# cxjyxxme/deep-online-video-stabilization

Measured on AMD Instinct MI355X. Metric: stabilized frames/sec (720p, before_ch=31), higher is better.
Workload: dtype f32 (bf16x3 split MFMA, f32 accumulate); 1 GPU; BASELINE.json configs[1]: v2_93 net, 1280x720, 1 stream(s)/GPU, batch=1 per stream, 13-ch stack from a 32-deep ring (lags 1,2,4,8,16,32; --before-ch 31 ignored as in the reference), ResNet-v2-50 regressor + 4x4 multi-grid warp + feedback; one independent stream set per GPU (replicas only); height=720, width=1280, streams_per_gpu=1, refine=1, operand_mode=4, launches_per_frame=64, hip_graph=True

## Files before the change

### deep-online-video-stabilization_amd/csrc/conv.hip

```cpp
#include "conv.h"
#include "prof.h"
#include <climits>
#include <cstdlib>
#include <algorithm>
#include <vector>

#include "conv_kernel.h"
#include "conv_ring_kernel.h"
#include "conv_b2b_kernel.h"

template <int PAIR>
__device__ __forceinline__ void conv_splitk_reduce_body(const ConvArgs& p, const ConvPair& pr) {
    const size_t q = (size_t)blockIdx.x * 256 + threadIdx.x;
    const int c4n = p.Cout / 4;
    if (q >= (size_t)p.M * c4n) return;
    const int m = (int)(q / c4n);
    const int n = (int)(q - (size_t)m * c4n) * 4;
    const bool t1 = PAIR && m >= pr.m_tower;
    const size_t slab = (size_t)p.M * p.Cout;
    const float* src = p.partial + (size_t)m * p.Cout + n;
    float4 s = *reinterpret_cast<const float4*>(src);
    for (int z = 1; z < p.splitk; ++z) {
        const float4 t = *reinterpret_cast<const float4*>(src + z * slab);
        s.x += t.x; s.y += t.y; s.z += t.z; s.w += t.w;
    }
    if (p.bias != nullptr) {
        const float4 b = *reinterpret_cast<const float4*>(p.bias + n);
        s.x += b.x; s.y += b.y; s.z += b.z; s.w += b.w;
    }
    if (p.residual != nullptr) {
        size_t ri;
        if (p.res_stride == 1 && p.res_H == p.Ho && p.res_W == p.Wo) {
            ri = (size_t)m * p.res_ld + n;
        } else {
            const int img = sn_fastdiv(m, p.div_hw_mul, p.div_hw_shift);
            const int rr = m - img * (p.Ho * p.Wo);
            const int oy = sn_fastdiv(rr, p.div_w_mul, p.div_w_shift), ox = rr - oy * p.Wo;
            ri = (((size_t)img * p.res_H + oy * p.res_stride) * p.res_W + ox * p.res_stride) * p.res_ld + n;
        }
        const float4 t = *reinterpret_cast<const float4*>(p.residual + (t1 ? pr.dres : 0) + ri);
        s.x += t.x; s.y += t.y; s.z += t.z; s.w += t.w;
    }
    if (p.out_scale != nullptr) {
        const float4 a = *reinterpret_cast<const float4*>(p.out_scale + n), b = *reinterpret_cast<const float4*>(p.out_shift + n);
        s.x = __builtin_fmaf(s.x, a.x, b.x); s.y = __builtin_fmaf(s.y, a.y, b.y);
        s.z = __builtin_fmaf(s.z, a.z, b.z); s.w = __builtin_fmaf(s.w, a.w, b.w);
    }
    if (p.out_scale != nullptr && p.out_floor != nullptr) {
        const float4 f = *reinterpret_cast<const float4*>(p.out_floor + n);
        s.x = fmaxf(s.x, f.x); s.y = fmaxf(s.y, f.y); s.z = fmaxf(s.z, f.z); s.w = fmaxf(s.w, f.w);
    } else if (p.relu_out) {
        s.x = fmaxf(s.x, 0.f); s.y = fmaxf(s.y, 0.f); s.z = fmaxf(s.z, 0.f); s.w = fmaxf(s.w, 0.f);
    }
    *reinterpret_cast<float4*>(p.y + (t1 ? pr.dy : 0) + (size_t)m * p.Cout + n) = s;
}
__global__ __launch_bounds__(256) void conv_splitk_reduce_kernel(const ConvArgs p) {
    conv_splitk_reduce_body<0>(p, ConvPair{});
}
__global__ __launch_bounds__(256) void conv_splitk_reduce_pair_kernel(const ConvArgs p, const ConvPair pr) {
    conv_splitk_reduce_body<1>(p, pr);
}

enum TileId { T128x128 = 0, T128x64 = 1, T64x64 = 2 };

static void tile_dims(int t, int& bm, int& bn) {
    bm = (t == T64x64) ? 64 : 128;
    bn = (t == T128x128) ? 128 : 64;
}

static int env_int(const char* name, int dflt) {
    const char* v = getenv(name);
    return v ? atoi(v) : dflt;
}

static int g_force_tile = -2, g_force_split = -1, g_force_bk16 = 0;

static int conv_bk(const ConvArgs& a) { return (a.rowrun || (a.Cin % 32 == 0 && !g_force_bk16)) ? 32 : 16; }
static int conv_total_steps(const ConvArgs& a) {
    if (a.rowrun) return a.KH * cdiv(a.KW * a.Cin, 32);
    return a.KH * a.KW * (a.Cin / conv_bk(a));
}

struct TuneEntry { int M, Cout, K, KH, ring, splitk; };
#include "conv_tuning_table.h"
#include "conv_tuning_table_packed.h"
static int g_tuning_profile = 0;
static std::vector<TuneEntry> g_tuning_runtime;
static int g_tuning_use_builtin = -1;

static int tuning_lookup(int M, int Cout, int K, int KH, int ring) {
    for (const TuneEntry& e : g_tuning_runtime)
        if (e.M == M && e.Cout == Cout && e.K == K && e.KH == KH && e.ring == ring) return e.splitk;
    if (g_tuning_use_builtin < 0) g_tuning_use_builtin = env_int("STABNET_CONV_TUNING_TABLE", 1);
    if (g_tuning_use_builtin && g_tuning_profile == 1)
        for (const TuneEntry& e : g_tuning_packed)
            if (e.M == M && e.Cout == Cout && e.K == K && e.KH == KH && e.ring == ring) return e.splitk;
    if (g_tuning_use_builtin)
        for (const TuneEntry& e : g_tuning_builtin)
            if (e.M == M && e.Cout == Cout && e.K == K && e.KH == KH && e.ring == ring) return e.splitk;
    return 0;
}

static int pick_tile(const ConvArgs& a, int& splitk) {
    if (g_force_tile == -2) {
        g_force_tile = env_int("STABNET_CONV_TILE", -1);
        g_force_split = env_int("STABNET_CONV_SPLITK", -1);
        g_force_bk16 = env_int("STABNET_CONV_BK16", 0);
    }
    const int force_tile = g_force_tile, force_split = g_force_split;
    if (force_tile >= 0) {
        const int steps0 = conv_total_steps(a);
        splitk = force_split > 0 ? std::min(force_split, steps0) : 1;
        return force_tile;
    }
    const int total_steps = conv_total_steps(a);
    const long blocks = (long)cdiv(a.M, 64) * cdiv(a.Cout, 64);
    const bool ring_path = a.rowrun || (a.in_scale_expected == 0 && a.up == 1 && a.Cin % 32 == 0);
    int s = tuning_lookup(a.M, a.Cout, a.K, a.KH, ring_path ? 1 : 0);
    static const int thr = env_int("STABNET_CONV_SPLIT_BELOW", 400), target = env_int("STABNET_CONV_SPLIT_TARGET", 448);
    if (s > 0) {
        s = std::min(s, std::max(1, total_steps / 2));
    } else if (blocks < thr && a.Cout % 4 == 0) {
        s = (int)((target + blocks / 2) / blocks);
        s = std::min(s, std::max(1, total_steps / 8));
        s = std::min(s, 32);
    } else {
        s = 1;
    }
    splitk = std::max(1, s);
    return T64x64;
}

size_t conv_plan(ConvArgs& a) {
    static const int swz = env_int("STABNET_CONV_XCD", 1);
    a.xcd_swizzle = swz;
    a.M = a.N * a.Ho * a.Wo;
    a.K = a.rowrun ? a.KH * 32 * cdiv(a.KW * a.Cin, 32) : a.KH * a.KW * a.Cin;
    if (a.x_ld == 0) a.x_ld = a.Cin;
    if (a.res_ld == 0) a.res_ld = a.Cout;
    sn_fastdiv_make((unsigned)(a.Ho * a.Wo), a.div_hw_mul, a.div_hw_shift);
    sn_fastdiv_make((unsigned)a.Wo, a.div_w_mul, a.div_w_shift);
    int splitk = 1;
    (void)pick_tile(a, splitk);
    const int total_steps = conv_total_steps(a);
    a.steps_per_split = cdiv(total_steps, splitk);
    a.splitk = cdiv(total_steps, a.steps_per_split);
    return a.splitk > 1 ? (size_t)a.splitk * a.M * a.Cout * sizeof(float) : 0;
}

template <int BM, int BN, int BK, int WM, int WN, int MODE, int NBUF, int BF16 = 0>
static int launch_one_nb(const ConvArgs& a, hipStream_t st) {
    constexpr size_t lds_op = NBUF * (size_t)(BM + BN) * (BK + 4) * sizeof(float);
    constexpr size_t lds_epi = 4 * (size_t)SN_EPI_WAVE_BYTES;
    constexpr size_t lds = lds_op > lds_epi ? lds_op : lds_epi;
    static bool configured = false;
    auto kern = conv_igemm_f32_kernel<BM, BN, BK, WM, WN, MODE, NBUF, BF16>;
    if (!configured) {
        if (lds > 64 * 1024) {
            hipError_t e = hipFuncSetAttribute(reinterpret_cast<const void*>(kern),
                                               hipFuncAttributeMaxDynamicSharedMemorySize, (int)lds);
            if (e != hipSuccess) {
                stabnet_set_error("conv: hipFuncSetAttribute(%zu B LDS) failed: %s", lds, hipGetErrorString(e));
                return STABNET_ERR_LAUNCH;
            }
        }
        configured = true;
    }
    dim3 grid(cdiv(a.M, BM), cdiv(a.Cout, BN), a.splitk);
    kern<<<grid, 256, lds, st>>>(a);
    SN_LAUNCH_CHECK("conv_igemm_f32_kernel");
    return STABNET_OK;
}

static thread_local int g_bf16_operands = 0;

static void igemm_variant(const ConvArgs& a, int bm, int bn, int bk, int mode, int& nbuf_out, int& bf16_out) {
    static const int nbuf = env_int("STABNET_CONV_NBUF", 0);
    bf16_out = (g_bf16_operands && bm == 64 && bn == 64 && bk == 32) ? g_bf16_operands : 0;
    const bool one_stage = nbuf == 1 || (nbuf == 0 && mode == 0 && bm == 64 && bn == 64 && a.M >= 32768);
    nbuf_out = (bf16_out != 1 && one_stage) ? 1 : 2;
}

template <int BM, int BN, int BK, int WM, int WN, int MODE>
static int launch_one_t(const ConvArgs& a, hipStream_t st) {
    int nbuf, bf16;
    igemm_variant(a, BM, BN, BK, MODE, nbuf, bf16);
    if constexpr (BM == 64 && BN == 64 && BK == 32) {
        if (bf16 == 1) return launch_one_nb<BM, BN, BK, WM, WN, MODE, 2, 1>(a, st);
        else if (bf16 == 2) return nbuf == 1 ? launch_one_nb<BM, BN, BK, WM, WN, MODE, 1, 2>(a, st) : launch_one_nb<BM, BN, BK, WM, WN, MODE, 2, 2>(a, st);
        else if (bf16 == 3) return nbuf == 1 ? launch_one_nb<BM, BN, BK, WM, WN, MODE, 1, 3>(a, st) : launch_one_nb<BM, BN, BK, WM, WN, MODE, 2, 3>(a, st);
    }
    return nbuf == 1 ? launch_one_nb<BM, BN, BK, WM, WN, MODE, 1>(a, st) : launch_one_nb<BM, BN, BK, WM, WN, MODE, 2>(a, st);
}

template <int BM, int BN, int BK, int WM, int WN>
static int launch_one(const ConvArgs& a, hipStream_t st) {
    if (a.up > 1) return launch_one_t<BM, BN, BK, WM, WN, 2>(a, st);
    if (a.pad == 0) return launch_one_t<BM, BN, BK, WM, WN, 0>(a, st);
    return launch_one_t<BM, BN, BK, WM, WN, 1>(a, st);
}

static int g_ring = -1;

static bool ring_eligible(const ConvArgs& a, int tile, bool has_prologue) {
    if (g_ring < 0) {
        g_ring = env_int("STABNET_CONV_RING", 1);
    }
    if (a.rowrun) return true;
    static const int lowk = env_int("STABNET_CONV_LOWK_IGEMM", 1);
    if (lowk && a.KH == 1 && a.KW == 1 && a.Cin == 64 && a.x_ld == a.Cin && a.out_floor == nullptr) return false;
    return g_ring && tile == T64x64 && !has_prologue && a.up == 1 && a.Cin % 32 == 0 && !g_force_bk16;
}
static bool ring_eligible(const ConvArgs& a, int tile) { return ring_eligible(a, tile, a.in_scale != nullptr); }

static int g_ring_wgs = 0;
static int g_ring_cus = 0;
static int g_reserved_cus = 0;
static int usable_cus(int cus) { return std::max(cus / 8, cus - std::max(0, g_reserved_cus)); }
static int ring_grid_cap() { return g_ring_cus > 0 ? g_ring_wgs / g_ring_cus * usable_cus(g_ring_cus) : g_ring_wgs; }

template <int MODE>
static int launch_ring_mode(const ConvArgs& a, hipStream_t st) {
    if (g_ring_wgs == 0) {
        int dev = 0, cus = 0;
        if (hipGetDevice(&dev) != hipSuccess || hipDeviceGetAttribute(&cus, hipDeviceAttributeMultiprocessorCount, dev) != hipSuccess ||
            cus <= 0) {
            stabnet_set_error("conv: cannot read the CU count");
            return STABNET_ERR_LAUNCH;
        }
        g_ring_wgs = env_int("STABNET_CONV_RING_WGS_PER_CU", 3) * cus;
        g_ring_cus = cus;
    }
    const long ntiles = (long)cdiv(a.M, 64) * cdiv(a.Cout, 64) * a.splitk;
    const int grid = (int)std::min<long>(ntiles, ring_grid_cap());
    if (g_bf16_operands == 1) conv_ring_f32_kernel<MODE, 1><<<grid, 256, 0, st>>>(a);
    else if (g_bf16_operands == 2) conv_ring_f32_kernel<MODE, 2><<<grid, 256, 0, st>>>(a);
    else if (g_bf16_operands == 3) conv_ring_f32_kernel<MODE, 3><<<grid, 256, 0, st>>>(a);
    else conv_ring_f32_kernel<MODE, 0><<<grid, 256, 0, st>>>(a);
    SN_LAUNCH_CHECK("conv_ring_f32_kernel");
    return STABNET_OK;
}

static int g_cus = 0;
static int device_cus() {
    if (g_cus == 0) {
        int dev = 0, cus = 0;
        if (hipGetDevice(&dev) != hipSuccess || hipDeviceGetAttribute(&cus, hipDeviceAttributeMultiprocessorCount, dev) != hipSuccess || cus <= 0)
            return 0;
        g_cus = cus;
    }
    return g_cus;
}

int conv_packed_variant() {
    static const int share = env_int("STABNET_CONV_PACKED_SHARE", 0);
    return share ? 5 : 4;
}

template <int MODE>
static int launch_ring_packed_mode(const ConvArgs& a, hipStream_t st) {
    const int cus = device_cus();
    if (cus <= 0) {
        stabnet_set_error("conv: cannot read the CU count");
        return STABNET_ERR_LAUNCH;
    }
    static const int per_cu = env_int("STABNET_CONV_PACKED_WGS_PER_CU", 2);
    const long ntiles = (long)cdiv(a.M, 64) * cdiv(a.Cout, 64) * a.splitk;
    const int grid = (int)std::min<long>(ntiles, (long)per_cu * usable_cus(cus));
    if constexpr (MODE == 0) {
        if (a.in_scale != nullptr) {
            if (conv_packed_variant() == 5) conv_ring_f32_kernel<0, 5, 1, 1><<<grid, 256, 0, st>>>(a);
            else conv_ring_f32_kernel<0, 4, 1, 1><<<grid, 256, 0, st>>>(a);
            SN_LAUNCH_CHECK("conv_ring_f32_kernel<packed, PRO>");
            return STABNET_OK;
        }
    }
    if (conv_packed_variant() == 5) conv_ring_f32_kernel<MODE, 5><<<grid, 256, 0, st>>>(a);
    else conv_ring_f32_kernel<MODE, 4><<<grid, 256, 0, st>>>(a);
    SN_LAUNCH_CHECK("conv_ring_f32_kernel<packed>");
    return STABNET_OK;
}
static int launch_ring_packed_kg2(const ConvArgs& a, hipStream_t st) {
    const int cus = device_cus();
    if (cus <= 0) {
        stabnet_set_error("conv: cannot read the CU count");
        return STABNET_ERR_LAUNCH;
    }
    const long ntiles = (long)cdiv(a.M, 64) * cdiv(a.Cout, 64);
    const int grid = (int)std::min<long>(ntiles, usable_cus(cus));
    if (conv_packed_variant() == 5) {
        if (a.in_scale != nullptr) conv_ring_f32_kernel<0, 5, 2, 1><<<grid, 512, 0, st>>>(a);
        else if (a.pad == 0) conv_ring_f32_kernel<0, 5, 2, 0><<<grid, 512, 0, st>>>(a);
        else conv_ring_f32_kernel<1, 5, 2, 0><<<grid, 512, 0, st>>>(a);
    } else {
        if (a.in_scale != nullptr) conv_ring_f32_kernel<0, 4, 2, 1><<<grid, 512, 0, st>>>(a);
        else if (a.pad == 0) conv_ring_f32_kernel<0, 4, 2, 0><<<grid, 512, 0, st>>>(a);
        else conv_ring_f32_kernel<1, 4, 2, 0><<<grid, 512, 0, st>>>(a);
    }
    SN_LAUNCH_CHECK("conv_ring_f32_kernel<packed, KG 2>");
    return STABNET_OK;
}
static int launch_ring_packed(const ConvArgs& a, hipStream_t st) {
    if (a.rowrun) return launch_ring_packed_mode<2>(a, st);
    return a.pad == 0 ? launch_ring_packed_mode<0>(a, st) : launch_ring_packed_mode<1>(a, st);
}

static int launch_ring(const ConvArgs& a, hipStream_t st) {
    if (a.rowrun) return launch_ring_mode<2>(a, st);
    return a.pad == 0 ? launch_ring_mode<0>(a, st) : launch_ring_mode<1>(a, st);
}

static bool ring_pro_vectors_ok(const ConvArgs& a) {
    if (a.in_scale == nullptr || a.in_shift == nullptr) return true;
    const long d = (long)(a.in_shift - a.in_scale);
    return d >= 0 && d < (1L << 30);
}
static bool ring_pro_geometry(const ConvArgs& a, bool has_prologue) {
    static const int on = env_int("STABNET_CONV_RING_PRO", 1);
    if (g_ring < 0) g_ring = env_int("STABNET_CONV_RING", 1);
    return on && g_ring && g_bf16_operands != 1 && !g_force_bk16 && has_prologue && a.KH == 1 && a.KW == 1 && a.stride == 1 && a.pad == 0 &&
           a.up == 1 && a.Cin % 32 == 0 && !a.rowrun && a.x_ld == a.Cin;
}
static int conv_kgroups(const ConvArgs& a, bool ring, bool has_prologue) {
    static const int on = env_int("STABNET_CONV_KGROUPS", 1);
    static const int on2 = env_int("STABNET_CONV_KGROUPS_PRO", 1);
    if (!on || a.splitk < 2 || g_bf16_operands == 1) return 1;
    const int steps = conv_total_steps(a);
    if (a.steps_per_split * a.splitk != steps) return 1;
    if (ring && a.splitk == 3 && !a.rowrun) return 3;
    if (on2 && !ring && a.splitk == 2 && ring_pro_geometry(a, has_prologue) && ring_pro_vectors_ok(a)) return 2;
    return 1;
}


static int launch_ring_kg(const ConvArgs& a, int kg, hipStream_t st) {
    const int cus = device_cus();
    if (cus <= 0) {
        stabnet_set_error("conv: cannot read the CU count");
        return STABNET_ERR_LAUNCH;
    }
    const long ntiles = (long)cdiv(a.M, 64) * cdiv(a.Cout, 64);
    const int grid = (int)std::min<long>(ntiles, usable_cus(cus));
#define SN_KG_LAUNCH(B)                                                                  \
    do {                                                                                  \
        if (kg == 2) conv_ring_f32_kernel<0, B, 2, 1><<<grid, 512, 0, st>>>(a);           \
        else if (a.pad == 0) conv_ring_f32_kernel<0, B, 3><<<grid, 768, 0, st>>>(a);      \
        else conv_ring_f32_kernel<1, B, 3><<<grid, 768, 0, st>>>(a);                      \
    } while (0)
    if (g_bf16_operands == 2) SN_KG_LAUNCH(2);
    else if (g_bf16_operands == 3) SN_KG_LAUNCH(3);
    else SN_KG_LAUNCH(0);
#undef SN_KG_LAUNCH
    SN_LAUNCH_CHECK("conv_ring_f32_kernel<KG>");
    return STABNET_OK;
}

static bool ring_pro_eligible(const ConvArgs& a) {
    static const int on = env_int("STABNET_CONV_RING_PRO", 1);
    if (g_ring < 0) g_ring = env_int("STABNET_CONV_RING", 1);
    return on && g_ring && g_bf16_operands != 1 && !g_force_bk16 && a.in_scale != nullptr && a.KH == 1 && a.KW == 1 && a.stride == 1 && a.pad == 0 &&
           a.up == 1 && a.Cin % 32 == 0 && a.out_scale == nullptr && a.out_floor == nullptr && !a.rowrun && a.x_ld == a.Cin &&
           ring_pro_vectors_ok(a);
}
static int launch_ring_pro(ConvArgs a, long delta, hipStream_t st) {
    if (g_ring_wgs == 0) {
        const int cus = device_cus();
        if (cus <= 0) {
            stabnet_set_error("conv: cannot read the CU count");
            return STABNET_ERR_LAUNCH;
        }
        g_ring_wgs = env_int("STABNET_CONV_RING_WGS_PER_CU", 3) * cus;
        g_ring_cus = cus;
    }
    a.out_floor = reinterpret_cast<const float*>((size_t)delta);
    const long ntiles = (long)cdiv(a.M, 64) * cdiv(a.Cout, 64) * a.splitk;
    const int grid = (int)std::min<long>(ntiles, ring_grid_cap());
    if (g_bf16_operands == 2) conv_ring_f32_kernel<0, 2, 1, 1><<<grid, 256, 0, st>>>(a);
    else if (g_bf16_operands == 3) conv_ring_f32_kernel<0, 3, 1, 1><<<grid, 256, 0, st>>>(a);
    else conv_ring_f32_kernel<0, 0, 1, 1><<<grid, 256, 0, st>>>(a);
    SN_LAUNCH_CHECK("conv_ring_f32_kernel<PRO>");
    return STABNET_OK;
}

int conv_reduce_launches(const ConvArgs& a, int operand_mode) {
    if (a.splitk < 2) return 0;
    int splitk_unused = 1;
    const int t = pick_tile(a, splitk_unused);
    const bool pro = a.in_scale_expected != 0;
    const bool ring = ring_eligible(a, t, pro);
    if (operand_mode == 4 && t == T64x64 && a.K % 32 == 0 && conv_bk(a) == 32) {
        static const int kg2_on = env_int("STABNET_CONV_PACKED_KG2", 1), pro_on = env_int("STABNET_CONV_PACKED_PRO", 1),
                         kg3_on = env_int("STABNET_CONV_PACKED_KG3", 1);
        const int kgf = conv_kgroups(a, ring, pro);
        const bool takes = (ring && (kgf == 1 || (kgf == 3 && kg3_on))) || (!ring && pro && pro_on && ring_pro_geometry(a, true));
        if (takes) return (kg2_on && a.splitk == 2 && !a.rowrun && a.steps_per_split * 2 == conv_total_steps(a)) ? 0 : 1;
    }
    return (t == T64x64 && conv_kgroups(a, ring, pro) > 1) ? 0 : 1;
}

size_t conv_weight_image_floats(int Cout, int K) { return (size_t)cdiv(Cout, 64) * (size_t)(K / 32) * 3072; }

__device__ __forceinline__ void weight_split_image_thread(const float* __restrict__ w, int Cout, int K, uint4* __restrict__ img, long i) {
    const int steps = K / 32;
    const int lane = (int)(i & 63), j = (int)((i >> 6) & 1), wn = (int)((i >> 7) & 1);
    const long ts = i >> 8;
    const int ks = (int)(ts % steps), nt = (int)(ts / steps);
    const int n = nt * 64 + wn * 32 + (lane & 31), g = lane >> 5;
    f32x4 lo = {0.f, 0.f, 0.f, 0.f}, hi = lo;
    if (n < Cout) {
        const float* r = w + (size_t)n * K + ks * 32 + 16 * j + 4 * g;
        lo = *reinterpret_cast<const f32x4*>(r);
        hi = *reinterpret_cast<const f32x4*>(r + 8);
    }
    const SnSplit3 a = sn_split3(lo), b = sn_split3(hi);
    uint4* out = img + ts * 768 + (size_t)(wn * 6 + j) * 64 + lane;
    out[0] = __builtin_bit_cast(uint4, SN_CAT8(a.h, b.h));
    out[2 * 64] = __builtin_bit_cast(uint4, SN_CAT8(a.m, b.m));
    out[4 * 64] = __builtin_bit_cast(uint4, SN_CAT8(a.l, b.l));
}

__global__ __launch_bounds__(256) void weight_split_image_kernel(const float* __restrict__ w, int Cout, int K, uint4* __restrict__ img) {
    const long i = (long)blockIdx.x * 256 + threadIdx.x;
    if (i >= (long)((Cout + 63) / 64) * (K / 32) * 256) return;
    weight_split_image_thread(w, Cout, K, img, i);
}

__global__ __launch_bounds__(256) void weight_split_images_kernel(const float* __restrict__ w_base, float* __restrict__ img_base, const WeightImageTable t) {
    const long i = (long)blockIdx.x * 256 + threadIdx.x;
    if (i >= t.tprefix[t.n]) return;
    int e = 0;
    while (i >= t.tprefix[e + 1]) ++e;
    weight_split_image_thread(w_base + t.w_off[e], t.Cout[e], t.K[e], reinterpret_cast<uint4*>(img_base + t.img_off[e]), i - t.tprefix[e]);
}

void weight_image_table_add(WeightImageTable& t, long w_off, long img_off, int Cout, int K) {
    if (t.n == 0) t.tprefix[0] = 0;
    t.w_off[t.n] = w_off; t.img_off[t.n] = img_off; t.Cout[t.n] = Cout; t.K[t.n] = K;
    t.tprefix[t.n + 1] = t.tprefix[t.n] + (long)cdiv(Cout, 64) * (K / 32) * 256;
    ++t.n;
}

int launch_weight_split_images(const float* w_base, float* img_base, const WeightImageTable& t, hipStream_t st) {
    if (t.n == 0) return STABNET_OK;
    SN_REQUIRE(w_base && img_base && t.n <= 64, "weight images: bad table");
    weight_split_images_kernel<<<(unsigned)(t.tprefix[t.n] >> 8), 256, 0, st>>>(w_base, img_base, t);
    SN_LAUNCH_CHECK("weight_split_images_kernel");
    return STABNET_OK;
}

int launch_weight_split_image(const float* w, int Cout, int K, float* img, hipStream_t st) {
    SN_REQUIRE(w && img && Cout > 0 && K > 0 && K % 32 == 0, "weight image: K=%d must be a multiple of 32", K);
    const long total = (long)cdiv(Cout, 64) * (K / 32) * 256;
    weight_split_image_kernel<<<cdiv(total, 256), 256, 0, st>>>(w, Cout, K, reinterpret_cast<uint4*>(img));
    SN_LAUNCH_CHECK("weight_split_image_kernel");
    return STABNET_OK;
}

int conv_launch(const ConvArgs& a_in, hipStream_t st, Prof* prof, int bf16_operands, const float* w_img) {
    const bool want_packed = bf16_operands == 4 && w_img != nullptr;
    if (bf16_operands == 4) bf16_operands = 0;
    g_bf16_operands = bf16_operands;
    const ConvArgs& a = a_in;
    SN_REQUIRE(a.rowrun || a.Cin % 16 == 0, "conv: Cin=%d must be a multiple of 16 (pad the channels)", a.Cin);
    SN_REQUIRE(!a.rowrun || (a.in_scale == nullptr && a.up == 1 && a.KH <= 8 && cdiv(a.KW * a.Cin, 32) <= 4),
               "conv: row-run operand needs no prologue, KH <= 8 and KW*Cin <= 128");
    SN_REQUIRE(a.Cout % 4 == 0, "conv: Cout=%d must be a multiple of 4", a.Cout);
    SN_REQUIRE(a.splitk >= 1 && a.steps_per_split >= 1 && a.div_hw_mul != 0, "conv: conv_plan() not called");
    SN_REQUIRE(a.splitk == 1 || a.partial != nullptr, "conv: split-K needs a workspace");
    int splitk_unused = 1;
    const int t = pick_tile(a, splitk_unused);
    const bool bk32 = conv_bk(a) == 32;
    int rc;
    const bool rec = prof != nullptr && prof->begin(st);
    const bool ring = ring_eligible(a, t);
    SN_REQUIRE(ring || a.x_ld == a.Cin, "conv: a strided input (x_ld %d != Cin %d) needs the ring kernel", a.x_ld, a.Cin);
    int kg = (t == T64x64) ? conv_kgroups(a, ring, a.in_scale != nullptr) : 1;
    static const int packed_kg3 = env_int("STABNET_CONV_PACKED_KG3", 1);
    if (want_packed && packed_kg3 && ring && kg == 3 && a.K % 32 == 0 && a.partial != nullptr) kg = 1;
    const bool pro = kg == 1 && !ring && t == T64x64 && bk32 && ring_pro_eligible(a);
    static const int packed_pro_on = env_int("STABNET_CONV_PACKED_PRO", 1);
    const bool packed_pro = want_packed && packed_pro_on && !ring && t == T64x64 && bk32 && a.in_scale != nullptr && a.out_floor == nullptr &&
                            ring_pro_geometry(a, true) && ring_pro_vectors_ok(a) && (a.splitk == 1 || a.partial != nullptr);
    if (packed_pro) kg = 1;
    const bool packed = (want_packed && ring && kg == 1 && !pro && a.K % 32 == 0) || packed_pro;
    static const int packed_kg2_on = env_int("STABNET_CONV_PACKED_KG2", 1);
    const bool packed_kg2 = packed && packed_kg2_on && a.splitk == 2 && !a.rowrun && a.steps_per_split * 2 == conv_total_steps(a);
    if (packed_kg2) kg = 2;
    if (packed) {
        ConvArgs b = a;
        b.w = w_img;
        rc = packed_kg2 ? launch_ring_packed_kg2(b, st) : launch_ring_packed(b, st);
    } else if (pro) {
        rc = launch_ring_pro(a, 0, st);
    } else if (kg > 1) {
        rc = launch_ring_kg(a, kg, st);
    } else if (ring) {
        rc = launch_ring(a, st);
    } else if (bk32) {
        if (t == T128x128) rc = launch_one<128, 128, 32, 64, 64>(a, st);
        else if (t == T128x64) rc = launch_one<128, 64, 32, 64, 32>(a, st);
        else rc = launch_one<64, 64, 32, 32, 32>(a, st);
    } else {
        if (t == T128x128) rc = launch_one<128, 128, 16, 64, 64>(a, st);
        else if (t == T128x64) rc = launch_one<128, 64, 16, 64, 32>(a, st);
        else rc = launch_one<64, 64, 16, 32, 32>(a, st);
    }
    const int mode = (a.up > 1 || a.rowrun) ? 2 : (a.pad == 0 ? 0 : 1);
    const bool b_has_pro = a.in_scale != nullptr;
    int kind = PK_KERNEL_CONV_RING + mode + (bf16_operands ? 3 : 0);
    if (packed) {
        kind = packed_kg2 ? (b_has_pro ? PK_KERNEL_CONV_PACKED + 6 : PK_KERNEL_CONV_PACKED + 4 + mode)
                          : (b_has_pro ? PK_KERNEL_CONV_PACKED + 3 : PK_KERNEL_CONV_PACKED + mode);
    } else if (pro) {
        kind = PK_KERNEL_CONV_KG + 2;
    } else if (kg > 1) {
        kind = kg == 2 ? PK_KERNEL_CONV_KG + 3 : PK_KERNEL_CONV_KG + mode;
    } else if (!ring) {
        int bm, bn, nbuf, bf16;
        tile_dims(t, bm, bn);
        igemm_variant(a, bm, bn, bk32 ? 32 : 16, mode, nbuf, bf16);
        kind = PK_KERNEL_CONV_BASE + mode * 6 + t * 2 + (bk32 ? 1 : 0) + (nbuf == 1 ? 18 : 0) + (bf16 ? 36 : 0);
    }
    if (rec) prof->end(st, kind, 2.0 * a.M * (double)(a.KH * a.KW * (a.cin_real ? a.cin_real : a.Cin)) * a.Cout,
                       4.0 * ((double)a.N * a.H * a.W * a.Cin + (double)a.K * a.Cout + (double)a.M * a.Cout * (kg > 1 ? 1 : a.splitk) +
                              ((a.residual != nullptr && (a.splitk == 1 || kg > 1)) ? (double)a.M * a.Cout : 0.0)),
                       a.M, a.Cout, a.K, a.splitk);
    if (rc) return rc;
    if (a.splitk > 1 && kg == 1) {
        const size_t q = (size_t)a.M * (a.Cout / 4);
        const bool rec2 = prof != nullptr && prof->begin(st);
        conv_splitk_reduce_kernel<<<cdiv((long)q, 256), 256, 0, st>>>(a);
        if (rec2) prof->end(st, PK_KERNEL_SPLITK_REDUCE, 0.0, 4.0 * (double)a.M * a.Cout * (a.splitk + 1 + (a.residual != nullptr ? 1 : 0)));
        SN_LAUNCH_CHECK("conv_splitk_reduce_kernel");
    }
    return STABNET_OK;
}

bool conv_pair_supported(const ConvArgs& a) {
    int splitk_unused = 1;
    const int t = pick_tile(a, splitk_unused);
    const bool pro = a.in_scale != nullptr || a.in_scale_expected;
    return t == T64x64 && !ring_eligible(a, t, pro) && a.up == 1 && !a.rowrun && (a.x_ld == 0 || a.x_ld == a.Cin);
}

template <int BK, int MODE>
static int launch_pair_one(const ConvArgs& a, const ConvPair& pr, hipStream_t st) {
    constexpr size_t lds = 2 * (size_t)(64 + 64) * (BK + 4) * sizeof(float);
    static_assert(lds >= 4 * (size_t)SN_EPI_WAVE_BYTES && lds <= 64 * 1024, "LDS of the 64x64 tile");
    dim3 grid(cdiv(a.M, 64), cdiv(a.Cout, 64), a.splitk);
    conv_igemm_f32_pair_kernel<64, 64, BK, 32, 32, MODE><<<grid, 256, lds, st>>>(a, pr);
    SN_LAUNCH_CHECK("conv_igemm_f32_pair_kernel");
    return STABNET_OK;
}

static int launch_ring_packed_pro_pair(ConvArgs a, long delta, const float* w_img, hipStream_t st) {
    const int cus = device_cus();
    if (cus <= 0) {
        stabnet_set_error("conv: cannot read the CU count");
        return STABNET_ERR_LAUNCH;
    }
    a.w = w_img;
    a.out_floor = reinterpret_cast<const float*>((size_t)delta);
    static const int per_cu = env_int("STABNET_CONV_PACKED_WGS_PER_CU", 2);
    const long ntiles = (long)cdiv(a.M, 64) * cdiv(a.Cout, 64) * a.splitk;
    const int grid = (int)std::min<long>(ntiles, (long)per_cu * usable_cus(cus));
    if (conv_packed_variant() == 5) conv_ring_f32_kernel<0, 5, 1, 1><<<grid, 256, 0, st>>>(a);
    else conv_ring_f32_kernel<0, 4, 1, 1><<<grid, 256, 0, st>>>(a);
    SN_LAUNCH_CHECK("conv_ring_f32_kernel<packed, PRO, pair>");
    return STABNET_OK;
}

int conv_launch_pair(const ConvArgs& a, const ConvPair& pr, hipStream_t st, Prof* prof, const float* w_img) {
    g_bf16_operands = 0;
    SN_REQUIRE(a.Cin % 16 == 0 && a.Cout % 4 == 0, "conv pair: Cin %% 16 and Cout %% 4 must be 0");
    SN_REQUIRE(a.splitk >= 1 && a.steps_per_split >= 1 && a.div_hw_mul != 0, "conv pair: conv_plan() not called");
    SN_REQUIRE(a.splitk == 1 || a.partial != nullptr, "conv pair: split-K needs a workspace");
    SN_REQUIRE(conv_pair_supported(a), "conv pair: the plan of this shape is not the 64x64 register-staged launch");
    SN_REQUIRE(pr.m_tower > 0 && pr.m_tower % 64 == 0 && a.M == 2 * pr.m_tower, "conv pair: tower rows %d must be a multiple of 64 (M %d)",
               pr.m_tower, a.M);
    const bool bk32 = conv_bk(a) == 32;
    const int mode = a.pad == 0 ? 0 : 1;
    const bool rec = prof != nullptr && prof->begin(st);
    int rc;
    const bool pro = bk32 && ring_pro_eligible(a) && pr.dx == pr.dscale - (long)pr.m_tower * a.Cin && pr.dy == pr.dscale - (long)pr.m_tower * a.Cout &&
                     (a.residual == nullptr || pr.dres == pr.dscale - (long)(a.N / 2) * a.res_H * a.res_W * a.res_ld);
    const bool packed = pro && w_img != nullptr && a.K % 32 == 0 && a.splitk == 1;
    if (packed) rc = launch_ring_packed_pro_pair(a, pr.dscale, w_img, st);
    else if (pro) rc = launch_ring_pro(a, pr.dscale, st);
    else if (bk32) rc = mode == 0 ? launch_pair_one<32, 0>(a, pr, st) : launch_pair_one<32, 1>(a, pr, st);
    else rc = mode == 0 ? launch_pair_one<16, 0>(a, pr, st) : launch_pair_one<16, 1>(a, pr, st);
    if (rec) prof->end(st, packed ? PK_KERNEL_CONV_PACKED + 3 : pro ? PK_KERNEL_CONV_KG + 2 : PK_KERNEL_CONV_PAIR + mode * 2 + (bk32 ? 1 : 0), 2.0 * a.M * (double)(a.KH * a.KW * (a.cin_real ? a.cin_real : a.Cin)) * a.Cout,
                       4.0 * ((double)a.N * a.H * a.W * a.Cin + (double)a.K * a.Cout + (double)a.M * a.Cout * a.splitk),
                       a.M, a.Cout, a.K, a.splitk);
    if (rc) return rc;
    if (a.splitk > 1) {
        const size_t q = (size_t)a.M * (a.Cout / 4);
        const bool rec2 = prof != nullptr && prof->begin(st);
        conv_splitk_reduce_pair_kernel<<<cdiv((long)q, 256), 256, 0, st>>>(a, pr);
        if (rec2) prof->end(st, PK_KERNEL_SPLITK_REDUCE, 0.0, 4.0 * (double)a.M * a.Cout * (a.splitk + 1));
        SN_LAUNCH_CHECK("conv_splitk_reduce_pair_kernel");
    }
    return STABNET_OK;
}

bool conv_b2b_supported(const ConvArgs& c2, const ConvArgs& c3) {
    static const int on = env_int("STABNET_CONV_B2B", 1);
    if (g_ring < 0) g_ring = env_int("STABNET_CONV_RING", 1);
    const bool g2 = c2.KH == 3 && c2.KW == 3 && c2.pad == 1 && c2.up == 1 && !c2.rowrun && (c2.stride == 1 || c2.stride == 2) &&
                    c2.Cin == c2.Cout && (c2.Cout == 64 || c2.Cout == 128) && c2.in_scale_expected == 0 && c2.in_scale == nullptr;
    const bool g3 = c3.KH == 1 && c3.KW == 1 && c3.pad == 0 && c3.stride == 1 && c3.up == 1 && !c3.rowrun && c3.Cin == c2.Cout &&
                    (c3.x_ld == 0 || c3.x_ld == c3.Cin) && c3.Cout % c2.Cout == 0 && c3.N == c2.N && c3.H == c2.Ho && c3.W == c2.Wo &&
                    c3.in_scale_expected == 0 && c3.in_scale == nullptr;
    return on && g_ring && g2 && g3;
}

int conv_b2b_launch(const ConvArgs& c2, const ConvArgs& c3, hipStream_t st, Prof* prof) {
    SN_REQUIRE(conv_b2b_supported(c2, c3), "conv b2b: unsupported geometry");
    SN_REQUIRE(c2.div_hw_mul != 0 && c3.div_hw_mul != 0 && c2.M == c3.M, "conv b2b: conv_plan() not called on both convolutions");
    SN_REQUIRE(c2.x && c2.w && c3.w && c3.y && c2.out_scale && c2.out_shift, "conv b2b: null pointer");
    SN_REQUIRE(c2.bias == nullptr && c2.residual == nullptr, "conv b2b: the 3x3 convolution takes no bias / residual");
    SN_REQUIRE(g_bf16_operands == 0, "conv b2b: fp32 only");
    const int cus = device_cus();
    if (cus <= 0) {
        stabnet_set_error("conv: cannot read the CU count");
        return STABNET_ERR_LAUNCH;
    }
    B2bArgs P;
    P.c2 = c2;
    P.c3 = c3;
    P.c3.splitk = 1;
    P.c3.steps_per_split = conv_total_steps(c3);
    const int tiles_m = cdiv(c2.M, 64);
    const bool rec = prof != nullptr && prof->begin(st);
    if (c2.Cout == 64) {
        static const int wgs = env_int("STABNET_CONV_B2B_WGS_PER_CU", 2);
        conv_b2b_f32_kernel<2><<<std::min(tiles_m, wgs * usable_cus(cus)), 256, 0, st>>>(P);
    } else {
        conv_b2b_f32_kernel<4><<<std::min(tiles_m, usable_cus(cus)), 512, 0, st>>>(P);
    }
    if (rec) prof->end(st, PK_KERNEL_CONV_B2B + (c2.Cout == 128 ? 1 : 0),
                       2.0 * c2.M * ((double)c2.K * c2.Cout + (double)c3.K * c3.Cout),
                       4.0 * ((double)c2.N * c2.H * c2.W * c2.Cin + (double)c2.K * c2.Cout + (double)c3.K * c3.Cout +
                              (double)c3.M * c3.Cout * (c3.residual ? 2 : 1)),
                       c2.M, c3.Cout, c2.K + c3.K, 1);
    SN_LAUNCH_CHECK("conv_b2b_f32_kernel");
    return STABNET_OK;
}

static int fill_args(ConvArgs& a, const float* x, const float* w, const float* bias, const float* in_scale,
                     const float* in_shift, const float* residual, int res_H, int res_W, int res_stride, float* y,
                     int N, int H, int W, int Cin, int Cout, int KH, int KW, int stride, int pad, int relu_out) {
    SN_REQUIRE(N > 0 && H > 0 && W > 0 && Cin > 0 && Cout > 0 && KH > 0 && KW > 0 && stride > 0 && pad >= 0,
               "conv2d: bad geometry");
    SN_REQUIRE(Cin % 16 == 0, "conv2d: Cin=%d must be a multiple of 16", Cin);
    SN_REQUIRE((in_scale == nullptr) == (in_shift == nullptr), "conv2d: in_scale and in_shift go together");
    a = ConvArgs{};
    a.x = x; a.w = w; a.y = y; a.bias = bias; a.in_scale = in_scale; a.in_shift = in_shift; a.residual = residual;
    a.in_scale_expected = in_scale != nullptr ? 1 : 0;
    a.N = N; a.H = H; a.W = W; a.Cin = Cin; a.Cout = Cout; a.KH = KH; a.KW = KW; a.stride = stride; a.pad = pad;
    a.up = 1;
    a.Ho = (H + 2 * pad - KH) / stride + 1;
    a.Wo = (W + 2 * pad - KW) / stride + 1;
    SN_REQUIRE(a.Ho > 0 && a.Wo > 0, "conv2d: empty output");
    a.res_H = residual ? res_H : a.Ho;
    a.res_W = residual ? res_W : a.Wo;
    a.res_stride = residual ? res_stride : 1;
    a.relu_out = relu_out;
    SN_REQUIRE((long)N * a.Ho * a.Wo * Cout < (1L << 30) && (long)N * (H + 2 * pad) * (W + 2 * pad) * Cin < (1L << 30) &&
                   (long)Cout * KH * KW * Cin < (1L << 30), "conv2d: tensors must have < 2^30 elements");
    SN_REQUIRE(KH * KW <= 64, "conv2d: filter larger than 64 taps");
    return STABNET_OK;
}

extern "C" {

int stabnet_conv_reserve_cus(int reserved) {
    const int prev = g_reserved_cus;
    g_reserved_cus = reserved < 0 ? 0 : reserved;
    return prev;
}

void stabnet_conv_tuning_override(int tile, int splitk) {
    g_force_tile = tile < 0 ? -1 : tile;
    g_force_split = splitk;
}

void stabnet_conv_tuning_profile(int profile) { g_tuning_profile = profile == 1 ? 1 : 0; }

void stabnet_conv_tuning_table_set(int M, int Cout, int K, int KH, int ring, int splitk) {
    if (M < 0) { g_tuning_runtime.clear(); return; }
    for (size_t i = 0; i < g_tuning_runtime.size(); ++i) {
        TuneEntry& e = g_tuning_runtime[i];
        if (e.M == M && e.Cout == Cout && e.K == K && e.KH == KH && e.ring == ring) {
            if (splitk > 0) e.splitk = splitk;
            else g_tuning_runtime.erase(g_tuning_runtime.begin() + i);
            return;
        }
    }
    if (splitk > 0) g_tuning_runtime.push_back({M, Cout, K, KH, ring, splitk});
}

size_t stabnet_conv2d_workspace_bytes(int N, int H, int W, int Cin, int Cout, int KH, int KW, int stride, int pad) {
    ConvArgs a;
    if (fill_args(a, nullptr, nullptr, nullptr, nullptr, nullptr, nullptr, 0, 0, 1, nullptr, N, H, W, Cin, Cout, KH, KW,
                  stride, pad, 0))
        return 0;
    ConvArgs b = a;
    b.in_scale_expected = 1;
    return std::max(conv_plan(a), conv_plan(b));
}

int stabnet_conv2d_fwd_ex(const float* x, const float* w_ohwi, const float* bias, const float* in_scale,
                          const float* in_shift, const float* residual, int res_H, int res_W, int res_stride,
                          const float* out_scale, const float* out_shift, float* y, int N, int H, int W, int Cin,
                          int Cout, int KH, int KW, int stride, int pad, int relu_out, void* workspace,
                          size_t workspace_bytes, void* stream);

int stabnet_conv2d_fwd(const float* x, const float* w_ohwi, const float* bias, const float* in_scale,
                       const float* in_shift, const float* residual, int res_H, int res_W, int res_stride, float* y,
                       int N, int H, int W, int Cin, int Cout, int KH, int KW, int stride, int pad, int relu_out,
                       void* workspace, size_t workspace_bytes, void* stream) {
    return stabnet_conv2d_fwd_ex(x, w_ohwi, bias, in_scale, in_shift, residual, res_H, res_W, res_stride, nullptr, nullptr,
                                 y, N, H, W, Cin, Cout, KH, KW, stride, pad, relu_out, workspace, workspace_bytes, stream);
}

int stabnet_conv2d_fwd_ex(const float* x, const float* w_ohwi, const float* bias, const float* in_scale,
                          const float* in_shift, const float* residual, int res_H, int res_W, int res_stride,
                          const float* out_scale, const float* out_shift, float* y, int N, int H, int W, int Cin,
                          int Cout, int KH, int KW, int stride, int pad, int relu_out, void* workspace,
                          size_t workspace_bytes, void* stream) {
    SN_REQUIRE(x && w_ohwi && y, "conv2d_fwd: null pointer");
    SN_REQUIRE((out_scale == nullptr) == (out_shift == nullptr), "conv2d_fwd: out_scale and out_shift go together");
    ConvArgs a;
    int rc = fill_args(a, x, w_ohwi, bias, in_scale, in_shift, residual, res_H, res_W, res_stride, y, N, H, W, Cin, Cout,
                       KH, KW, stride, pad, relu_out);
    if (rc) return rc;
    const size_t need = conv_plan(a);
    if (need > workspace_bytes || (need > 0 && workspace == nullptr)) {
        stabnet_set_error("conv2d_fwd: workspace %zu B < %zu B needed", workspace_bytes, need);
        return STABNET_ERR_WORKSPACE;
    }
    a.partial = static_cast<float*>(workspace);
    a.out_scale = out_scale;
    a.out_shift = out_shift;
    return conv_launch(a, (hipStream_t)stream);
}

size_t stabnet_conv_weight_image_floats(int Cout, int KH, int KW, int Cin) {
    const int K = KH * KW * Cin;
    return (Cout > 0 && K > 0 && K % 32 == 0) ? conv_weight_image_floats(Cout, K) : 0;
}

int stabnet_conv_weight_split_image(const float* w_ohwi, int Cout, int KH, int KW, int Cin, float* w_img, void* stream) {
    SN_REQUIRE(w_ohwi && w_img, "conv_weight_split_image: null pointer");
    SN_REQUIRE(Cin % 32 == 0, "conv_weight_split_image: Cin=%d must be a multiple of 32", Cin);
    return launch_weight_split_image(w_ohwi, Cout, KH * KW * Cin, w_img, (hipStream_t)stream);
}

int stabnet_conv2d_fwd_packed(const float* x, const float* w_ohwi, const float* w_img, const float* bias, const float* in_scale,
                              const float* in_shift, const float* residual, int res_H, int res_W, int res_stride,
                              const float* out_scale, const float* out_shift, float* y, int N, int H, int W, int Cin,
                              int Cout, int KH, int KW, int stride, int pad, int relu_out, int splitk, void* workspace,
                              size_t workspace_bytes, void* stream) {
    SN_REQUIRE(x && w_ohwi && w_img && y, "conv2d_fwd_packed: null pointer");
    SN_REQUIRE((out_scale == nullptr) == (out_shift == nullptr), "conv2d_fwd_packed: out_scale and out_shift go together");
    ConvArgs a;
    int rc = fill_args(a, x, w_ohwi, bias, in_scale, in_shift, residual, res_H, res_W, res_stride, y, N, H, W, Cin, Cout,
                       KH, KW, stride, pad, relu_out);
    if (rc) return rc;
    size_t need = conv_plan(a);
    if (splitk > 0) {
        const int total = conv_total_steps(a);
        a.steps_per_split = cdiv(total, std::min(splitk, total));
        a.splitk = cdiv(total, a.steps_per_split);
        need = a.splitk > 1 ? (size_t)a.splitk * a.M * a.Cout * sizeof(float) : 0;
    }
    if (need > workspace_bytes || (need > 0 && workspace == nullptr)) {
        stabnet_set_error("conv2d_fwd_packed: workspace %zu B < %zu B needed", workspace_bytes, need);
        return STABNET_ERR_WORKSPACE;
    }
    a.partial = static_cast<float*>(workspace);
    a.out_scale = out_scale;
    a.out_shift = out_shift;
    return conv_launch(a, (hipStream_t)stream, nullptr, 4, w_img);
}

int stabnet_conv3x3_conv1x1_fwd(const float* x, int x_ld, const float* w2_ohwi, const float* mid_scale, const float* mid_shift,
                                const float* w3_ohwi, const float* bias3, const float* residual, int res_H, int res_W,
                                int res_stride, int res_ld, const float* out_scale, const float* out_shift, float* y, int N, int H,
                                int W, int C, int Cout, int stride, int relu_out, void* stream) {
    SN_REQUIRE(x && w2_ohwi && mid_scale && mid_shift && w3_ohwi && y, "conv3x3_conv1x1_fwd: null pointer");
    SN_REQUIRE((out_scale == nullptr) == (out_shift == nullptr), "conv3x3_conv1x1_fwd: out_scale and out_shift go together");
    ConvArgs c2, c3;
    int rc = fill_args(c2, x, w2_ohwi, nullptr, nullptr, nullptr, nullptr, 0, 0, 1, nullptr, N, H, W, C, C, 3, 3, stride, 1, 1);
    if (rc) return rc;
    c2.x_ld = x_ld;
    (void)conv_plan(c2);
    c2.out_scale = mid_scale;
    c2.out_shift = mid_shift;
    rc = fill_args(c3, nullptr, w3_ohwi, bias3, nullptr, nullptr, residual, res_H, res_W, res_stride, y, N, c2.Ho, c2.Wo, C, Cout,
                   1, 1, 1, 0, relu_out);
    if (rc) return rc;
    c3.res_ld = res_ld;
    (void)conv_plan(c3);
    c3.out_scale = out_scale;
    c3.out_shift = out_shift;
    SN_REQUIRE(conv_b2b_supported(c2, c3), "conv3x3_conv1x1_fwd: C must be 64 or 128, Cout a multiple of C, stride 1 or 2");
    g_bf16_operands = 0;
    return conv_b2b_launch(c2, c3, (hipStream_t)stream);
}

}
```

### deep-online-video-stabilization_amd/csrc/conv_ring_kernel.h

```cpp
#pragma once
#include "conv_kernel.h"
#include <type_traits>

#ifndef RING_ABLATE
#define RING_ABLATE 0
#endif

typedef __attribute__((address_space(3))) void* sn_lds_ptr_t;
typedef const __attribute__((address_space(1))) void* sn_gbl_ptr_t;

__device__ __attribute__((aligned(16))) float g_conv_zero_page[8];

#ifndef RING_STAMP
#define RING_STAMP 0
#endif
#if RING_STAMP
__device__ unsigned long long g_ring_stamps[4096 * 8];
#define SN_STAMP(i) do { if (threadIdx.x == 0 && blockIdx.x < 4096) g_ring_stamps[blockIdx.x * 8 + (i)] = __builtin_amdgcn_s_memrealtime(); } while (0)
#define SN_STAMP_RT(i) do { if (threadIdx.x == 0 && blockIdx.x < 4096) g_ring_stamps[blockIdx.x * 8 + (i)] = __builtin_amdgcn_s_memrealtime(); } while (0)
#else
#define SN_STAMP(i) do { } while (0)
#define SN_STAMP_RT(i) do { } while (0)
#endif

template <int MODE ,
          int BF16 = 0 ,
          int KG = 1 ,
          int PRO = 0 >
__global__ __launch_bounds__(256 * KG) void conv_ring_f32_kernel(const ConvArgs p) {
    constexpr int BM = 64, BN = 64, BK = 32;
    constexpr bool PK = (BF16 >= 4);
    constexpr bool PS = (BF16 == 5);

    constexpr int B_STAGE = PK ? 3072 : BN * BK;
    constexpr int STAGE = BM * BK + B_STAGE;
    constexpr int PLANE_FLOATS = (BF16 == 5) ? 3072 : 0;
    constexpr int GROUP_FLOATS = 3 * STAGE + PLANE_FLOATS;
    static_assert(!PRO || (MODE == 0 && BF16 != 1), "the fragment prologue exists for the 1x1 fp32 / split kernels");
    static_assert(!PK || KG <= 2, "the packed split kernel splits K inside the workgroup two ways at most (60 KiB of ring per group)");
    constexpr int SC_FLOATS = PRO ? 3 * 4 * 64 : 0;
    __shared__ __attribute__((aligned(16))) float ring[KG * GROUP_FLOATS + KG * SC_FLOATS];

    const int tid = threadIdx.x, lane = tid & 63, wave = (KG > 1) ? ((tid >> 6) & 3) : (tid >> 6);
    const int grp = (KG > 1) ? __builtin_amdgcn_readfirstlane(tid >> 8) : 0;
    SN_STAMP(0); SN_STAMP_RT(4);
    const int wm = wave >> 1, wn = wave & 1;
    const int tiles_m = (p.M + BM - 1) / BM, tiles_n = (p.Cout + BN - 1) / BN;
    const int tiles_mn = tiles_m * tiles_n;
    const int ntiles = (KG > 1) ? tiles_mn : tiles_mn * p.splitk;
    int t_first = blockIdx.x, t_stride = gridDim.x, t_end = ntiles;
    if (p.xcd_swizzle && gridDim.x >= 8) {
        const int x = blockIdx.x & 7, Gt = (int)gridDim.x;
        t_stride = (Gt - x + 7) >> 3;
        const int before = x * (Gt >> 3) + min(x, Gt & 7);
        const int lo = (int)((long)ntiles * before / Gt), hi = (int)((long)ntiles * (before + t_stride) / Gt);
        t_first = lo + (blockIdx.x >> 3);
        t_end = hi;
    }
    const int cin_steps = (MODE == 2) ? 1 : p.Cin / BK;
    const int run_steps = (MODE == 2) ? p.K / (p.KH * BK) : 0;
    const int total_steps = (MODE == 2) ? p.K / BK : p.KH * p.KW * cin_steps;
    const int last_slice_steps = total_steps - (p.splitk - 1) * p.steps_per_split;
    const unsigned lds_base = (unsigned)(size_t)(sn_lds_ptr_t)ring + (KG > 1 ? (unsigned)grp * (unsigned)(GROUP_FLOATS * 4) : 0u);

    const long pair_delta = (PRO && KG == 1) ? (long)(size_t)p.out_floor : 0L;
    const int m_tower = (PRO && KG == 1 && pair_delta != 0) ? (p.M >> 1) : 0x7fffffff;
    const unsigned sc_base = (KG > 1) ? (unsigned)(size_t)(sn_lds_ptr_t)ring + (unsigned)(KG * GROUP_FLOATS * 4) + (unsigned)grp * (unsigned)(SC_FLOATS * 4)
                                      : lds_base + (unsigned)(GROUP_FLOATS * 4);
    int remaining = 0;
    for (int t = t_first; t < t_end; t += t_stride) remaining += (t / tiles_mn == p.splitk - 1) ? last_slice_steps : p.steps_per_split;

    const int rr = lane >> 3, cp = lane & 7;
    const int ld = p.x_ld;
    const int pad_off = (p.pad * p.W + p.pad) * ld;
    const int row_jump = (p.W - p.KW) * ld;
    const float* const zero_page = g_conv_zero_page;

    int pt = t_first;
    int p_left = 0;
    unsigned a_voff[2], w_voff[2];
    unsigned long long a_mask[2];
    int l_tap = 0, l_c0 = 0, l_kw = 0;
    const float *xb = p.x, *wb = p.w;
    const float* scb = p.in_scale;
    const unsigned sc_voff = PRO ? (unsigned)((lane & 31) * 4) + ((lane >> 5) ? (unsigned)((p.in_shift - p.in_scale) * 4) : 0u) : 0u;
    auto producer_setup = [&]() {
        const int z = (KG > 1) ? grp : pt / tiles_mn;
        const int mn = (KG > 1) ? pt : pt - z * tiles_mn;
        const int mt = mn / tiles_n, nt = mn - mt * tiles_n;
        const int m0 = mt * BM, n0 = nt * BN;
        const int ks_begin = z * p.steps_per_split;
        p_left = (z == p.splitk - 1) ? last_slice_steps : p.steps_per_split;
        if constexpr (MODE == 2) {
            const int Wp = p.W + 2 * p.pad, Hp = p.H + 2 * p.pad;
#pragma unroll
            for (int t = 0; t < 2; ++t) {
                const int row = 8 * (wave + 4 * t) + rr;
                const int cl = cp ^ ((row >> 1) & 7);
                const int mc = min(m0 + row, p.M - 1);
                const int img = sn_fastdiv(mc, p.div_hw_mul, p.div_hw_shift);
                const int r = mc - img * (p.Ho * p.Wo);
                const int oy = sn_fastdiv(r, p.div_w_mul, p.div_w_shift), ox = r - oy * p.Wo;
                a_voff[t] = 4u * (unsigned)(((img * Hp + oy * p.stride) * Wp + ox * p.stride) * p.Cin + cl * 4);
                a_mask[t] = 0;
                const int n = min(n0 + row, p.Cout - 1);
                w_voff[t] = 4u * (unsigned)(n * p.K + cl * 4);
            }
        } else {
#pragma unroll
            for (int t = 0; t < 2; ++t) {
                const int row = 8 * (wave + 4 * t) + rr;
                const int cl = cp ^ ((row >> 1) & 7);
                const int m = m0 + row;
                const int mc = min(m, p.M - 1);
                const int img = sn_fastdiv(mc, p.div_hw_mul, p.div_hw_shift);
                const int r = mc - img * (p.Ho * p.Wo);
                const int oy = sn_fastdiv(r, p.div_w_mul, p.div_w_shift), ox = r - oy * p.Wo;
                const int iy0 = oy * p.stride - p.pad, ix0 = ox * p.stride - p.pad;
                a_voff[t] = 4u * (unsigned)(((img * p.H + iy0 + p.pad) * p.W + ix0 + p.pad) * ld + cl * 4);
                unsigned long long mk = 0;
                if (MODE == 1 && m < p.M) {
                    const int kh_lo = max(0, -iy0), kh_hi = min(p.KH, p.H - iy0);
                    const int kw_lo = max(0, -ix0), kw_hi = min(p.KW, p.W - ix0);
                    if (kh_hi > kh_lo && kw_hi > kw_lo) {
                        const unsigned long long rowbits = ((1ull << (kw_hi - kw_lo)) - 1ull) << kw_lo;
                        for (int kh = kh_lo; kh < kh_hi; ++kh) mk |= rowbits << (kh * p.KW);
                    }
                }
                a_mask[t] = mk;
                const int n = min(n0 + row, p.Cout - 1);
                w_voff[t] = 4u * (unsigned)(n * p.K + cl * 4);
            }
        }
        if constexpr (MODE == 2) {
            l_tap = ks_begin / run_steps;
            l_kw = ks_begin - l_tap * run_steps;
            xb = p.x + ((long)l_tap * (p.W + 2 * p.pad) * p.Cin + 32 * l_kw);
            wb = PK ? p.w + ((size_t)nt * total_steps + ks_begin) * B_STAGE : p.w + (size_t)ks_begin * BK;
        } else {
            l_tap = ks_begin / cin_steps;
            l_c0 = (ks_begin - l_tap * cin_steps) * BK;
            const int l_kh = l_tap / p.KW;
            l_kw = l_tap - l_kh * p.KW;
            xb = p.x + ((l_kh * p.W + l_kw) * ld + l_c0 - pad_off);
            wb = PK ? p.w + ((size_t)nt * total_steps + ks_begin) * B_STAGE : p.w + (l_tap * p.Cin + l_c0);
            if constexpr (PRO) {
                const bool t2 = m0 >= m_tower;
                if (t2) xb += pair_delta - (long)m_tower * ld;
                scb = p.in_scale + l_c0 + (t2 ? pair_delta : 0L);
            }
        }
    };
    const unsigned dma_base = (unsigned)__builtin_amdgcn_readfirstlane((int)(lds_base + (unsigned)wave * 1024u));
    auto dma16 = [&](const float* base_, unsigned voff_bytes, unsigned lds_byte) {
        const unsigned long long b64 = (unsigned long long)(size_t)base_;
        const unsigned lo = (unsigned)__builtin_amdgcn_readfirstlane((int)(unsigned)b64);
        const unsigned hi = (unsigned)__builtin_amdgcn_readfirstlane((int)(unsigned)(b64 >> 32));
        const float* base = reinterpret_cast<const float*>((size_t)(((unsigned long long)hi << 32) | lo));
        if constexpr (PK) lds_byte = (unsigned)__builtin_amdgcn_readfirstlane((int)lds_byte);
        asm volatile("s_mov_b32 m0, %2\n\tglobal_load_lds_dwordx4 %0, %1" ::"v"(voff_bytes), "s"(base), "s"(lds_byte) : "memory", "m0");
    };
    auto issue_s = [&](int slot) {
        if (pt >= t_end) return;
        const unsigned long long b64 = (unsigned long long)(size_t)scb;
        const unsigned lo = (unsigned)__builtin_amdgcn_readfirstlane((int)(unsigned)b64);
        const unsigned hi = (unsigned)__builtin_amdgcn_readfirstlane((int)(unsigned)(b64 >> 32));
        const float* base = reinterpret_cast<const float*>((size_t)(((unsigned long long)hi << 32) | lo));
        const unsigned lds_byte = (unsigned)__builtin_amdgcn_readfirstlane((int)(sc_base + (unsigned)(slot * 1024 + wave * 256)));
        asm volatile("s_mov_b32 m0, %2\n\tglobal_load_lds_dword %0, %1" ::"v"(sc_voff), "s"(base), "s"(lds_byte) : "memory", "m0");
    };
    auto issue_a = [&](int slot, int t) {
        if (pt >= t_end || (RING_ABLATE & 1)) return;
        const unsigned lds_byte = dma_base + (unsigned)(slot * STAGE * 4 + t * 4096);
        if constexpr (MODE == 1) {
            const float* src = ((a_mask[t] >> l_tap) & 1ull) ? reinterpret_cast<const float*>(reinterpret_cast<const char*>(xb) + a_voff[t]) : zero_page;
            __builtin_amdgcn_global_load_lds((sn_gbl_ptr_t)src, (sn_lds_ptr_t)(size_t)lds_byte, 16, 0, 0);
        } else {
            dma16(xb, a_voff[t], lds_byte);
        }
    };
    const unsigned wimg_voff = (unsigned)(wave * 1024 + lane * 16);
    auto issue_b = [&](int slot, int t) {
        if (pt >= t_end || (RING_ABLATE & 1)) return;
        if constexpr (PK) dma16(wb, wimg_voff + (unsigned)(t * 4096), dma_base + (unsigned)(slot * STAGE * 4 + BM * BK * 4 + t * 4096));
        else dma16(wb, w_voff[t], dma_base + (unsigned)(slot * STAGE * 4 + BM * BK * 4 + t * 4096));
    };
    auto issue_advance = [&]() {
        if (pt >= t_end) return;
        if (--p_left == 0) {
            pt += t_stride;
            if (pt < t_end) producer_setup();
            return;
        }
        xb += BK;
        wb += PK ? B_STAGE : BK;
        if constexpr (PRO) scb += BK;
        if constexpr (MODE == 2) {
            if (++l_kw == run_steps) { l_kw = 0; ++l_tap; xb += (p.W + 2 * p.pad) * p.Cin - BK * run_steps; }
            return;
        }
        l_c0 += BK;
        if (l_c0 == p.Cin) {
            l_c0 = 0;
            ++l_tap;
            xb += ld - p.Cin;
            if (++l_kw == p.KW) { l_kw = 0; xb += row_jump; }
        }
    };
    auto issue_part = [&](int slot, int part) {
        if (part == 0) issue_a(slot, 0);
        else if (part == 1) { issue_a(slot, 1); issue_b(slot, 0); }
        else if (part == 2) { issue_b(slot, 1); if constexpr (PK) issue_b(slot, 2); if constexpr (PRO) issue_s(slot); }
        else issue_advance();
    };
    auto issue = [&](int slot) {
        issue_part(slot, 0); issue_part(slot, 1); issue_part(slot, 2); issue_part(slot, 3);
    };

    int ct = t_first, c_left = 0, c_m0 = 0, c_n0 = 0, c_z = 0;
    long c_yoff = 0, c_roff = 0;
    auto consumer_setup = [&]() {
        c_z = (KG > 1) ? grp : ct / tiles_mn;
        const int mn = (KG > 1) ? ct : ct - c_z * tiles_mn;
        const int mt = mn / tiles_n;
        c_m0 = mt * BM;
        c_n0 = (mn - mt * tiles_n) * BN;
        c_left = (c_z == p.splitk - 1) ? last_slice_steps : p.steps_per_split;
        if constexpr (PRO) {
            const bool t2 = c_m0 >= m_tower;
            c_yoff = t2 ? pair_delta - (long)m_tower * p.Cout : 0L;
            c_roff = t2 ? pair_delta - (long)(p.N >> 1) * p.res_H * p.res_W * p.res_ld : 0L;
        }
    };

    unsigned a_frag[4], b_frag[4];
    {
        const int ra = wm * 32 + (lane & 31), rb = wn * 32 + (lane & 31), h = lane >> 5;
#pragma unroll
        for (int kk = 0; kk < 4; ++kk) {
            a_frag[kk] = lds_base + 4 * (ra * BK + (((2 * kk + h) ^ ((ra >> 1) & 7)) << 2));
            b_frag[kk] = lds_base + 4 * (BM * BK + rb * BK + (((2 * kk + h) ^ ((rb >> 1) & 7)) << 2));
        }
    }

    f32x16 acc[1][1];
#pragma unroll
    for (int r = 0; r < 16; ++r) acc[0][0][r] = 0.f;

    if (remaining == 0) return;
    producer_setup();
    consumer_setup();

#define SN_RA0 "{v[100:103]}"
#define SN_RB0 "{v[104:107]}"
#define SN_RA1 "{v[108:111]}"
#define SN_RB1 "{v[112:115]}"
#define SN_DS_READ(dst, reg, addr, off)                                                                   \
    do { if (!(RING_ABLATE & 4)) asm volatile("ds_read_b128 %0, %1 offset:%2" : "=" reg(dst) : "v"(addr), "n"(off)); } while (0)
#define SN_READ0(kk, off) do { SN_DS_READ(a0, SN_RA0, a_frag[kk], off); SN_DS_READ(b0, SN_RB0, b_frag[kk], off); } while (0)
#define SN_READ1(kk, off) do { SN_DS_READ(a1, SN_RA1, a_frag[kk], off); SN_DS_READ(b1, SN_RB1, b_frag[kk], off); } while (0)
#define SN_WAIT0() asm volatile("s_waitcnt lgkmcnt(0)" : "+" SN_RA0(a0), "+" SN_RB0(b0))
#define SN_WAIT1() asm volatile("s_waitcnt lgkmcnt(0)" : "+" SN_RA1(a1), "+" SN_RB1(b1))
#define SN_PH0 "{v[132:135]}"
#define SN_PM0 "{v[136:139]}"
#define SN_PL0 "{v[140:143]}"
#define SN_PH1 "{v[144:147]}"
#define SN_PM1 "{v[148:151]}"
#define SN_PL1 "{v[152:155]}"
#define SN_READA(dst, reg, kk, off) SN_DS_READ(dst, reg, a_frag[kk], off)
#define SN_READB0(off) do { SN_DS_READ(ph0, SN_PH0, bimg_frag, (off) + 0); SN_DS_READ(pm0, SN_PM0, bimg_frag, (off) + 2048); SN_DS_READ(pl0, SN_PL0, bimg_frag, (off) + 4096); } while (0)
#define SN_READB1(off) do { SN_DS_READ(ph1, SN_PH1, bimg_frag, (off) + 1024); SN_DS_READ(pm1, SN_PM1, bimg_frag, (off) + 3072); SN_DS_READ(pl1, SN_PL1, bimg_frag, (off) + 5120); } while (0)
#define SN_RA2 "{v[156:159]}"
#define SN_RA3 "{v[160:163]}"
#define SN_RS2 "{v[164:167]}"
#define SN_RH2 "{v[168:171]}"
#define SN_RS3 "{v[172:175]}"
#define SN_RH3 "{v[176:179]}"
#define SN_WAIT_A01(n)                                                                                                     \
    do {                                                                                                                   \
        if constexpr (PRO) asm volatile("s_waitcnt lgkmcnt(" #n ")" : "+" SN_RA0(a0), "+" SN_RA1(a1), "+" SN_RS0(sc0), "+" SN_RH0(sh0), "+" SN_RS1(sc1), "+" SN_RH1(sh1)); \
        else asm volatile("s_waitcnt lgkmcnt(" #n ")" : "+" SN_RA0(a0), "+" SN_RA1(a1));                                  \
    } while (0)
#define SN_WAIT_A23B0(n)                                                                                                   \
    do {                                                                                                                   \
        if constexpr (PRO) asm volatile("s_waitcnt lgkmcnt(" #n ")" : "+" SN_RA2(a2), "+" SN_RA3(a3), "+" SN_PH0(ph0), "+" SN_PM0(pm0), "+" SN_PL0(pl0), "+" SN_RS2(sc2), "+" SN_RH2(sh2), "+" SN_RS3(sc3), "+" SN_RH3(sh3)); \
        else asm volatile("s_waitcnt lgkmcnt(" #n ")" : "+" SN_RA2(a2), "+" SN_RA3(a3), "+" SN_PH0(ph0), "+" SN_PM0(pm0), "+" SN_PL0(pl0)); \
    } while (0)
#define SN_READS8(soff)                                                                                                    \
    do {                                                                                                                   \
        if constexpr (PRO) {                                                                                               \
            SN_DS_READ(sc0, SN_RS0, s_frag[0], soff); SN_DS_READ(sh0, SN_RH0, s_frag[0], (soff) + 128);                    \
            SN_DS_READ(sc1, SN_RS1, s_frag[1], soff); SN_DS_READ(sh1, SN_RH1, s_frag[1], (soff) + 128);                    \
            SN_DS_READ(sc2, SN_RS2, s_frag[2], soff); SN_DS_READ(sh2, SN_RH2, s_frag[2], (soff) + 128);                    \
            SN_DS_READ(sc3, SN_RS3, s_frag[3], soff); SN_DS_READ(sh3, SN_RH3, s_frag[3], (soff) + 128);                    \
        }                                                                                                                  \
    } while (0)
#define SN_WAIT_B1() asm volatile("s_waitcnt lgkmcnt(0)" : "+" SN_PH1(ph1), "+" SN_PM1(pm1), "+" SN_PL1(pl1))
#define SN_READA4(off) do { SN_READA(a0, SN_RA0, 0, off); SN_READA(a1, SN_RA1, 1, off); SN_READA(a2, SN_RA2, 2, off); SN_READA(a3, SN_RA3, 3, off); } while (0)
#define SN_SB() __builtin_amdgcn_sched_barrier(0)
#define SN_PMFMA(ap, breg) do { if (!(RING_ABLATE & 8)) acc[0][0] = __builtin_amdgcn_mfma_f32_32x32x16_bf16(__builtin_bit_cast(sn_bf16x8, ap), __builtin_bit_cast(sn_bf16x8, breg), acc[0][0], 0, 0, 0); else acc[0][0][0] += __builtin_bit_cast(float, ap.x) + breg.x; SN_SB(); } while (0)
#define SN_L1(P, c, x0, x1) do { if (!(RING_ABLATE & 32)) P.h.c = sn_split_level(x0, x1); else P.h.c = __builtin_bit_cast(unsigned, x0); } while (0)
#define SN_L2(P, c, x0, x1) do { if (!(RING_ABLATE & 32)) P.m.c = sn_split_level(x0, x1); else P.m.c = __builtin_bit_cast(unsigned, x1); } while (0)
#define SN_L3(P, c, x0, x1) do { if (!(RING_ABLATE & 32)) P.l.c = sn_pack_bf16(x0, x1); else P.l.c = __builtin_bit_cast(unsigned, x0); } while (0)
#define SN_QH0 "{v[156:159]}"
#define SN_QM0 "{v[160:163]}"
#define SN_QL0 "{v[164:167]}"
#define SN_QH1 "{v[168:171]}"
#define SN_QM1 "{v[172:175]}"
#define SN_QL1 "{v[176:179]}"
#define SN_READQ()                                                                                                        \
    do {                                                                                                                  \
        SN_DS_READ(qh0, SN_QH0, pl_rd0, 0); SN_DS_READ(qm0, SN_QM0, pl_rd0, 1024); SN_DS_READ(ql0, SN_QL0, pl_rd0, 2048);  \
        SN_DS_READ(qh1, SN_QH1, pl_rd1, 0); SN_DS_READ(qm1, SN_QM1, pl_rd1, 1024); SN_DS_READ(ql1, SN_QL1, pl_rd1, 2048);  \
    } while (0)
#define SN_WAIT_Q0B0(n) asm volatile("s_waitcnt lgkmcnt(" #n ")" : "+" SN_QH0(qh0), "+" SN_QM0(qm0), "+" SN_QL0(ql0), "+" SN_PH0(ph0), "+" SN_PM0(pm0), "+" SN_PL0(pl0))
#define SN_WAIT_Q1B1() asm volatile("s_waitcnt lgkmcnt(0)" : "+" SN_QH1(qh1), "+" SN_QM1(qm1), "+" SN_QL1(ql1), "+" SN_PH1(ph1), "+" SN_PM1(pm1), "+" SN_PL1(pl1))
#define SN_READOWN(off, soff)                                                                                             \
    do {                                                                                                                  \
        if constexpr (PRO) {                                                                                              \
            SN_DS_READ(sc0, SN_RS0, s_own0, soff); SN_DS_READ(sh0, SN_RH0, s_own0, (soff) + 128);                          \
            SN_DS_READ(sc1, SN_RS1, s_own1, soff); SN_DS_READ(sh1, SN_RH1, s_own1, (soff) + 128);                          \
        }                                                                                                                 \
        SN_DS_READ(a0, SN_RA0, a_own0, off); SN_DS_READ(a1, SN_RA1, a_own1, off);                                          \
    } while (0)
#define SN_WRITEQ(P)                                                                                                      \
    do {                                                                                                                  \
        asm volatile("ds_write_b128 %0, %1" ::"v"(pl_wr), "v"(P.h) : "memory");                                           \
        asm volatile("ds_write_b128 %0, %1 offset:1024" ::"v"(pl_wr), "v"(P.m) : "memory");                               \
        asm volatile("ds_write_b128 %0, %1 offset:2048" ::"v"(pl_wr), "v"(P.l) : "memory");                               \
    } while (0)
#define SN_PS_GROUP0(OFF_)                                                                                               \
    asm volatile("s_waitcnt lgkmcnt(0)" ::: "memory");                     \
    SN_BARRIER();                                                                      \
    SN_READQ(); SN_READB1(OFF_);                                                                                         \
    SN_WAIT_Q0B0(6);                                            \
    SN_SB();                                                                                                             \
    SN_PMFMA(ql0, ph0); SN_PMFMA(qh0, pl0); SN_PMFMA(qm0, pm0); SN_PMFMA(qm0, ph0); SN_PMFMA(qh0, pm0); SN_PMFMA(qh0, ph0)
#define SN_PS_GROUP1_TAIL()                                                                                              \
    SN_WAIT_A01(3);                                         \
    if constexpr (PRO) { SN_PRO(a0, sc0, sh0); SN_PRO(a1, sc1, sh1); }                                                   \
    float y0 = a0.x, y1 = a0.y, y2 = a0.z, y3 = a0.w, y4 = a1.x, y5 = a1.y, y6 = a1.z, y7 = a1.w;                        \
    SnPlanes NP;                                                                                                         \
    SN_SB();                                                                                                             \
    SN_PMFMA(qm1, pm1); SN_L1(NP, x, y0, y1); SN_L1(NP, y, y2, y3); SN_SB();                                             \
    SN_PMFMA(qm1, ph1); SN_L1(NP, z, y4, y5); SN_L1(NP, w, y6, y7); SN_SB();                                             \
    SN_PMFMA(qh1, pm1); SN_L2(NP, x, y0, y1); SN_L2(NP, y, y2, y3); SN_SB();                                             \
    SN_PMFMA(qh1, ph1); SN_L2(NP, z, y4, y5); SN_L2(NP, w, y6, y7);                                                      \
    SN_L3(NP, x, y0, y1); SN_L3(NP, y, y2, y3); SN_L3(NP, z, y4, y5); SN_L3(NP, w, y6, y7); SN_SB();                     \
    SN_WRITEQ(NP); SN_SB()
#define SN_PK_GROUP0(OFF_)                                                                                               \
    SN_READB1(OFF_);                                                 \
    SN_WAIT_A23B0(3);                                                                                                    \
    if constexpr (PRO) { SN_PRO(a2, sc2, sh2); SN_PRO(a3, sc3, sh3); }                                                   \
    float x0 = a2.x, x1 = a2.y, x2 = a2.z, x3 = a2.w, x4 = a3.x, x5 = a3.y, x6 = a3.z, x7 = a3.w;                        \
    SN_SB();                                                                                                             \
    SN_PMFMA(AP.l, ph0); SN_L1(CP, x, x0, x1); SN_L1(CP, y, x2, x3); SN_SB();                                            \
    SN_PMFMA(AP.h, pl0); SN_L1(CP, z, x4, x5); SN_L1(CP, w, x6, x7); SN_SB();                                            \
    SN_PMFMA(AP.m, pm0); SN_L2(CP, x, x0, x1); SN_L2(CP, y, x2, x3); SN_SB();                                            \
    SN_PMFMA(AP.m, ph0); SN_L2(CP, z, x4, x5); SN_L2(CP, w, x6, x7); SN_SB();                                            \
    SN_PMFMA(AP.h, pm0); SN_L3(CP, x, x0, x1); SN_L3(CP, y, x2, x3); SN_L3(CP, z, x4, x5); SN_L3(CP, w, x6, x7); SN_SB(); \
    SN_PMFMA(AP.h, ph0)
#define SN_PK_GROUP1_TAIL()                                                                                              \
    SN_WAIT_A01(5);                                         \
    if constexpr (PRO) { SN_PRO(a0, sc0, sh0); SN_PRO(a1, sc1, sh1); }                                                   \
    float y0 = a0.x, y1 = a0.y, y2 = a0.z, y3 = a0.w, y4 = a1.x, y5 = a1.y, y6 = a1.z, y7 = a1.w;                        \
    SN_SB();                                                                                                             \
    SN_PMFMA(CP.m, pm1); SN_L1(AP, x, y0, y1); SN_L1(AP, y, y2, y3); SN_SB();                                            \
    SN_PMFMA(CP.m, ph1); SN_L1(AP, z, y4, y5); SN_L1(AP, w, y6, y7); SN_SB();                                            \
    SN_PMFMA(CP.h, pm1); SN_L2(AP, x, y0, y1); SN_L2(AP, y, y2, y3); SN_SB();                                            \
    SN_PMFMA(CP.h, ph1); SN_L2(AP, z, y4, y5); SN_L2(AP, w, y6, y7);                                                     \
    SN_L3(AP, x, y0, y1); SN_L3(AP, y, y2, y3); SN_L3(AP, z, y4, y5); SN_L3(AP, w, y6, y7); SN_SB()
#define SN_RS0 "{v[116:119]}"
#define SN_RH0 "{v[120:123]}"
#define SN_RS1 "{v[124:127]}"
#define SN_RH1 "{v[128:131]}"
#define SN_READ0P(kk, off, soff)                                                                      \
    do { SN_READ0(kk, off); SN_DS_READ(sc0, SN_RS0, s_frag[kk], soff); SN_DS_READ(sh0, SN_RH0, s_frag[kk], (soff) + 128); } while (0)
#define SN_READ1P(kk, off, soff)                                                                      \
    do { SN_READ1(kk, off); SN_DS_READ(sc1, SN_RS1, s_frag[kk], soff); SN_DS_READ(sh1, SN_RH1, s_frag[kk], (soff) + 128); } while (0)
#define SN_WAIT0P() asm volatile("s_waitcnt lgkmcnt(0)" : "+" SN_RA0(a0), "+" SN_RB0(b0), "+" SN_RS0(sc0), "+" SN_RH0(sh0))
#define SN_WAIT1P() asm volatile("s_waitcnt lgkmcnt(0)" : "+" SN_RA1(a1), "+" SN_RB1(b1), "+" SN_RS1(sc1), "+" SN_RH1(sh1))
#define SN_PRO(a, sc, sh)                                                                             \
    do {                                                                                              \
        a.x = fmaxf(__builtin_fmaf(a.x, sc.x, sh.x), 0.f); a.y = fmaxf(__builtin_fmaf(a.y, sc.y, sh.y), 0.f); \
        a.z = fmaxf(__builtin_fmaf(a.z, sc.z, sh.z), 0.f); a.w = fmaxf(__builtin_fmaf(a.w, sc.w, sh.w), 0.f); \
        __builtin_amdgcn_sched_barrier(0);                                                            \
    } while (0)
#define SN_MFMA1(a, b, c)                                                                                      \
    do {                                                                                                       \
        if (!(RING_ABLATE & 8)) acc[0][0] = __builtin_amdgcn_mfma_f32_32x32x2f32(a.c, b.c, acc[0][0], 0, 0, 0); \
        else acc[0][0][0] += a.c * b.c;                                                                        \
        __builtin_amdgcn_sched_barrier(0);                                                                     \
    } while (0)
#define SN_BARRIER()                                                     \
    do {                                                                 \
        if (!(RING_ABLATE & 2)) __builtin_amdgcn_s_barrier();            \
        __builtin_amdgcn_sched_barrier(0);                               \
    } while (0)

    f32x4 a0, b0, a1, b1;
    f32x4 sc0, sh0, sc1, sh1;
    f32x4 ph0, pm0, pl0, ph1, pm1, pl1;
    f32x4 a2, a3;
    f32x4 sc2, sh2, sc3, sh3;
    SnPlanes AP, CP;
    f32x4 qh0, qm0, ql0, qh1, qm1, ql1;
    const unsigned pl_base = lds_base + (unsigned)(3 * STAGE * 4);
    const unsigned pl_rd0 = pl_base + (unsigned)((wm * 2 + 0) * 3072 + lane * 16), pl_rd1 = pl_base + (unsigned)((wm * 2 + 1) * 3072 + lane * 16);
    const unsigned pl_wr = pl_base + (unsigned)((wm * 2 + wn) * 3072 + lane * 16);
    unsigned a_own0 = 0u, a_own1 = 0u, s_own0 = 0u, s_own1 = 0u;
    const unsigned bimg_frag = lds_base + (unsigned)(4 * BM * BK + wn * 6144 + lane * 16);
    unsigned s_frag[4] = {0u, 0u, 0u, 0u};
    if constexpr (PRO) {
#pragma unroll
        for (int kk = 0; kk < 4; ++kk) s_frag[kk] = sc_base + (unsigned)(wave * 256 + (8 * kk + 4 * (lane >> 5)) * 4);
    }
    if constexpr (PS) {
        const int ra = wm * 32 + (lane & 31), h = lane >> 5;
        a_own0 = lds_base + 4 * (ra * BK + (((2 * (2 * wn) + h) ^ ((ra >> 1) & 7)) << 2));
        a_own1 = lds_base + 4 * (ra * BK + (((2 * (2 * wn + 1) + h) ^ ((ra >> 1) & 7)) << 2));
        if constexpr (PRO) {
            s_own0 = sc_base + (unsigned)(wave * 256 + (8 * (2 * wn) + 4 * h) * 4);
            s_own1 = sc_base + (unsigned)(wave * 256 + (8 * (2 * wn + 1) + 4 * h) * 4);
        }
    }
    if (RING_ABLATE & 4) { a0 = b0 = a1 = b1 = f32x4{1.f, 2.f, 3.f, 4.f}; }
    issue(0);
    issue(1);
    if (remaining > 1) { if constexpr (PRO && PK) asm volatile("s_waitcnt vmcnt(6)" ::: "memory"); else if constexpr (PRO || PK) asm volatile("s_waitcnt vmcnt(5)" ::: "memory"); else asm volatile("s_waitcnt vmcnt(4)" ::: "memory"); }
    else asm volatile("s_waitcnt vmcnt(0)" ::: "memory");
    SN_BARRIER();
    SN_STAMP(1);
    issue(2);
    if constexpr (PS) {
        SN_READOWN(0, 0); SN_READB0(0);
        SN_WAIT_A01(3);
        if constexpr (PRO) { SN_PRO(a0, sc0, sh0); SN_PRO(a1, sc1, sh1); }
        const SnPlanes NP0 = sn_split3_pair(a0, a1);
        SN_SB();
        SN_WRITEQ(NP0);
        SN_SB();
    } else if constexpr (PK) {
        SN_READS8(0); SN_READA4(0); SN_READB0(0);
        SN_WAIT_A01(5);
        if constexpr (PRO) { SN_PRO(a0, sc0, sh0); SN_PRO(a1, sc1, sh1); }
        AP = sn_split3_pair(a0, a1);
        SN_SB();
    } else if constexpr (PRO) SN_READ0P(0, 0, 0); else SN_READ0(0, 0);

    auto step = [&](auto slot_c) -> bool {
        constexpr int SLOT = decltype(slot_c)::value;
        constexpr int OFF = SLOT * STAGE * 4;
        constexpr int OFF_NEXT = ((SLOT + 1) % 3) * STAGE * 4;
        bool tile_done, more;
        if constexpr (PS) {
            constexpr int SOFF_NEXT = ((SLOT + 1) % 3) * 1024;
            SN_PS_GROUP0(OFF);
            --remaining;
            tile_done = (--c_left == 0);
            more = remaining > 0;
            const bool feed = more && !tile_done;
            SN_WAIT_Q1B1();
            if (more) {
                if (remaining > 1) { if constexpr (PRO) asm volatile("s_waitcnt vmcnt(6)" ::: "memory"); else asm volatile("s_waitcnt vmcnt(5)" ::: "memory"); }
                else asm volatile("s_waitcnt vmcnt(0)" ::: "memory");
                SN_BARRIER();
            }
            SN_READOWN(OFF_NEXT, SOFF_NEXT); SN_READB0(OFF_NEXT);
            SN_PMFMA(ql1, ph1);
            if (feed) { issue_part(SLOT, 0); issue_part(SLOT, 1); SN_SB(); }
            SN_PMFMA(qh1, pl1);
            if (feed) { issue_part(SLOT, 2); issue_part(SLOT, 3); SN_SB(); }
            SN_PS_GROUP1_TAIL();
        } else if constexpr (PK) {
            SN_PK_GROUP0(OFF);
            --remaining;
            tile_done = (--c_left == 0);
            more = remaining > 0;
            const bool feed = more && !tile_done;
            SN_WAIT_B1();
            if (more) {
                if (remaining > 1) { if constexpr (PRO) asm volatile("s_waitcnt vmcnt(6)" ::: "memory"); else asm volatile("s_waitcnt vmcnt(5)" ::: "memory"); }
                else asm volatile("s_waitcnt vmcnt(0)" ::: "memory");
                SN_BARRIER();
            }
            SN_READS8(((SLOT + 1) % 3) * 1024); SN_READA4(OFF_NEXT); SN_READB0(OFF_NEXT);
            SN_PMFMA(CP.l, ph1);
            if (feed) { issue_part(SLOT, 0); issue_part(SLOT, 1); SN_SB(); }
            SN_PMFMA(CP.h, pl1);
            if (feed) { issue_part(SLOT, 2); issue_part(SLOT, 3); SN_SB(); }
            SN_PK_GROUP1_TAIL();
        } else if constexpr (BF16 >= 2) {
            constexpr int NPROD = (BF16 == 3) ? 9 : 6;
            constexpr int SOFF = SLOT * 1024, SOFF_NEXT = ((SLOT + 1) % 3) * 1024;
            if constexpr (PRO) { SN_WAIT0P(); SN_PRO(a0, sc0, sh0); } else SN_WAIT0();
            const SnSplit3 A0 = sn_split3(a0), B0 = sn_split3(b0);
            if constexpr (PRO) SN_READ1P(1, OFF, SOFF); else SN_READ1(1, OFF);
            if constexpr (PRO) { SN_WAIT1P(); SN_PRO(a1, sc1, sh1); } else SN_WAIT1();
            const SnSplit3 A1 = sn_split3(a1), B1 = sn_split3(b1);
            if constexpr (PRO) { SN_READ0P(2, OFF, SOFF); SN_READ1P(3, OFF, SOFF); } else { SN_READ0(2, OFF); SN_READ1(3, OFF); }
            sn_mfma_split3<NPROD>(acc[0][0], A0, A1, B0, B1);
            if constexpr (PRO) { SN_WAIT0P(); SN_WAIT1P(); SN_PRO(a0, sc0, sh0); SN_PRO(a1, sc1, sh1); }
            else { SN_WAIT0(); SN_WAIT1(); }
            const SnSplit3 C0 = sn_split3(a0), D0 = sn_split3(b0);
            const SnSplit3 C1 = sn_split3(a1), D1 = sn_split3(b1);
            __builtin_amdgcn_sched_barrier(0);
            --remaining;
            tile_done = (--c_left == 0);
            more = remaining > 0;
            const bool feed = more && !tile_done;
            if (more) {
                if (remaining > 1) { if constexpr (PRO) asm volatile("s_waitcnt vmcnt(5)" ::: "memory"); else asm volatile("s_waitcnt vmcnt(4)" ::: "memory"); }
                else asm volatile("s_waitcnt vmcnt(0)" ::: "memory");
                SN_BARRIER();
                if constexpr (PRO) SN_READ0P(0, OFF_NEXT, SOFF_NEXT); else SN_READ0(0, OFF_NEXT);
            }
            if (feed) { issue_part(SLOT, 0); issue_part(SLOT, 1); issue_part(SLOT, 2); issue_part(SLOT, 3); __builtin_amdgcn_sched_barrier(0); }
            sn_mfma_split3<NPROD>(acc[0][0], C0, C1, D0, D1);
            __builtin_amdgcn_sched_barrier(0);
        } else if constexpr (BF16) {
            SN_WAIT0();
            const sn_bf16x4 al = __builtin_convertvector(a0, sn_bf16x4), bl = __builtin_convertvector(b0, sn_bf16x4);
            SN_READ1(1, OFF);
            SN_WAIT1();
            const sn_bf16x4 ah = __builtin_convertvector(a1, sn_bf16x4), bh = __builtin_convertvector(b1, sn_bf16x4);
            SN_READ0(2, OFF);
            SN_READ1(3, OFF);
            acc[0][0] = __builtin_amdgcn_mfma_f32_32x32x16_bf16(__builtin_shufflevector(al, ah, 0, 1, 2, 3, 4, 5, 6, 7),
                                                                __builtin_shufflevector(bl, bh, 0, 1, 2, 3, 4, 5, 6, 7), acc[0][0], 0, 0, 0);
            __builtin_amdgcn_sched_barrier(0);
            SN_WAIT0();
            SN_WAIT1();
            const sn_bf16x4 cl = __builtin_convertvector(a0, sn_bf16x4), dl = __builtin_convertvector(b0, sn_bf16x4);
            const sn_bf16x4 ch = __builtin_convertvector(a1, sn_bf16x4), dh = __builtin_convertvector(b1, sn_bf16x4);
            __builtin_amdgcn_sched_barrier(0);
            --remaining;
            tile_done = (--c_left == 0);
            more = remaining > 0;
            const bool feed = more && !tile_done;
            if (more) {
                if (remaining > 1) asm volatile("s_waitcnt vmcnt(4)" ::: "memory");
                else asm volatile("s_waitcnt vmcnt(0)" ::: "memory");
                SN_BARRIER();
                SN_READ0(0, OFF_NEXT);
            }
            if (feed) { issue_part(SLOT, 0); issue_part(SLOT, 1); issue_part(SLOT, 2); issue_part(SLOT, 3); __builtin_amdgcn_sched_barrier(0); }
            acc[0][0] = __builtin_amdgcn_mfma_f32_32x32x16_bf16(__builtin_shufflevector(cl, ch, 0, 1, 2, 3, 4, 5, 6, 7),
                                                                __builtin_shufflevector(dl, dh, 0, 1, 2, 3, 4, 5, 6, 7), acc[0][0], 0, 0, 0);
            __builtin_amdgcn_sched_barrier(0);
        } else if constexpr (PRO) {
        constexpr int SOFF = SLOT * 1024, SOFF_NEXT = ((SLOT + 1) % 3) * 1024;
        SN_WAIT0P();
        SN_PRO(a0, sc0, sh0);
        SN_MFMA1(a0, b0, x);
        SN_READ1P(1, OFF, SOFF);
        SN_MFMA1(a0, b0, y);
        SN_MFMA1(a0, b0, z);
        SN_WAIT1P();
        SN_PRO(a1, sc1, sh1);
        SN_MFMA1(a0, b0, w);
        SN_MFMA1(a1, b1, x);
        SN_READ0P(2, OFF, SOFF);
        SN_MFMA1(a1, b1, y);
        SN_MFMA1(a1, b1, z);
        SN_WAIT0P();
        SN_PRO(a0, sc0, sh0);
        SN_MFMA1(a1, b1, w);
        SN_MFMA1(a0, b0, x);
        SN_READ1P(3, OFF, SOFF);
        SN_MFMA1(a0, b0, y);
        SN_MFMA1(a0, b0, z);
        SN_WAIT1P();
        SN_PRO(a1, sc1, sh1);
        SN_MFMA1(a0, b0, w);
        SN_MFMA1(a1, b1, x);
        --remaining;
        tile_done = (--c_left == 0);
        more = remaining > 0;
        const bool feed = more && !tile_done;
        if (more) {
            if (remaining > 1) asm volatile("s_waitcnt vmcnt(5)" ::: "memory");
            else asm volatile("s_waitcnt vmcnt(0)" ::: "memory");
            SN_BARRIER();
            SN_READ0P(0, OFF_NEXT, SOFF_NEXT);
        }
        if (feed) { issue_part(SLOT, 0); __builtin_amdgcn_sched_barrier(0); }
        SN_MFMA1(a1, b1, y);
        if (feed) { issue_part(SLOT, 1); __builtin_amdgcn_sched_barrier(0); }
        SN_MFMA1(a1, b1, z);
        if (feed) { issue_part(SLOT, 2); __builtin_amdgcn_sched_barrier(0); }
        SN_MFMA1(a1, b1, w);
        if (feed) { issue_part(SLOT, 3); __builtin_amdgcn_sched_barrier(0); }
        } else {
        SN_WAIT0();
        SN_MFMA1(a0, b0, x);
        SN_READ1(1, OFF);
        SN_MFMA1(a0, b0, y);
        SN_MFMA1(a0, b0, z);
        SN_MFMA1(a0, b0, w);
        SN_WAIT1();
        SN_MFMA1(a1, b1, x);
        SN_READ0(2, OFF);
        SN_MFMA1(a1, b1, y);
        SN_MFMA1(a1, b1, z);
        SN_MFMA1(a1, b1, w);
        SN_WAIT0();
        SN_MFMA1(a0, b0, x);
        SN_READ1(3, OFF);
        SN_MFMA1(a0, b0, y);
        SN_MFMA1(a0, b0, z);
        SN_MFMA1(a0, b0, w);
        SN_WAIT1();
        SN_MFMA1(a1, b1, x);
        --remaining;
        tile_done = (--c_left == 0);
        more = remaining > 0;
        const bool feed = more && !tile_done;
        if (more) {
            if (!(RING_ABLATE & 16)) {
                if (remaining > 1) asm volatile("s_waitcnt vmcnt(4)" ::: "memory");
                else asm volatile("s_waitcnt vmcnt(0)" ::: "memory");
            }
            SN_BARRIER();
            SN_READ0(0, OFF_NEXT);
        }
        if (feed) { issue_part(SLOT, 0); __builtin_amdgcn_sched_barrier(0); }
        SN_MFMA1(a1, b1, y);
        if (feed) { issue_part(SLOT, 1); __builtin_amdgcn_sched_barrier(0); }
        SN_MFMA1(a1, b1, z);
        if (feed) { issue_part(SLOT, 2); __builtin_amdgcn_sched_barrier(0); }
        SN_MFMA1(a1, b1, w);
        if (feed) { issue_part(SLOT, 3); __builtin_amdgcn_sched_barrier(0); }
        }
        if (tile_done) {
            if constexpr (PS) { asm volatile("s_waitcnt lgkmcnt(0)" : "+" SN_PH0(ph0), "+" SN_PM0(pm0), "+" SN_PL0(pl0)); if (!more) SN_BARRIER(); }
            else if constexpr (PK) { SN_WAIT_A23B0(0); if (!more) SN_BARRIER(); }
            else if (more) { if constexpr (PRO) SN_WAIT0P(); else SN_WAIT0(); }
            else SN_BARRIER();
            SN_STAMP(2);
            if constexpr (KG > 1) {
                const unsigned red = lds_base + (unsigned)(OFF + wave * 4096 + lane * 16);
                if (grp > 0) {
#pragma unroll
                    for (int q = 0; q < 4; ++q) {
                        const f32x4 v = {acc[0][0][4 * q], acc[0][0][4 * q + 1], acc[0][0][4 * q + 2], acc[0][0][4 * q + 3]};
                        asm volatile("ds_write_b128 %0, %1 offset:%2" ::"v"(red), "v"(v), "n"(q * 1024) : "memory");
                    }
                    asm volatile("s_waitcnt lgkmcnt(0)" ::: "memory");
                }
                SN_BARRIER();
                if (grp == 0) {
#pragma unroll
                    for (int g = 1; g < KG; ++g) {
                        f32x4 t0, t1, t2, t3;
                        const unsigned src = red + (unsigned)(g * GROUP_FLOATS * 4);
                        asm volatile("ds_read_b128 %0, %4 offset:0\n\tds_read_b128 %1, %4 offset:1024\n\t"
                                     "ds_read_b128 %2, %4 offset:2048\n\tds_read_b128 %3, %4 offset:3072\n\ts_waitcnt lgkmcnt(0)"
                                     : "=&v"(t0), "=&v"(t1), "=&v"(t2), "=&v"(t3) : "v"(src) : "memory");
#pragma unroll
                        for (int e = 0; e < 4; ++e) {
                            acc[0][0][e] += t0[e]; acc[0][0][4 + e] += t1[e]; acc[0][0][8 + e] += t2[e]; acc[0][0][12 + e] += t3[e];
                        }
                    }
                    conv_epilogue<1, 1, true>(acc, p, c_m0 + wm * 32, c_n0 + wn * 32, lane, 0,
                                              lds_base + (unsigned)(OFF + wave * SN_EPI_WAVE_BYTES));
                }
            } else if constexpr (PRO)
            conv_epilogue<1, 1, false, true>(acc, p, c_m0 + wm * 32, c_n0 + wn * 32, lane, c_z,
                                             lds_base + (unsigned)(OFF + wave * SN_EPI_WAVE_BYTES), c_yoff, c_roff);
            else
            conv_epilogue<1, 1>(acc, p, c_m0 + wm * 32, c_n0 + wn * 32, lane, c_z,
                                lds_base + (unsigned)(OFF + wave * SN_EPI_WAVE_BYTES));
#if RING_STAMP
            asm volatile("s_waitcnt vmcnt(0)" ::: "memory");
            SN_STAMP(3); SN_STAMP_RT(5);
#endif
#pragma unroll
            for (int r = 0; r < 16; ++r) acc[0][0][r] = 0.f;
            ct += t_stride;
            if (ct < t_end) consumer_setup();
            if (more) {
                SN_BARRIER();
                issue(SLOT);
            }
        }
        return more;
    };
    auto fast_step = [&](auto slot_c) {
        constexpr int SLOT = decltype(slot_c)::value;
        constexpr int OFF = SLOT * STAGE * 4;
        constexpr int OFF_NEXT = ((SLOT + 1) % 3) * STAGE * 4;
        if constexpr (PK) {
            if constexpr (PS) {
                SN_PS_GROUP0(OFF);
                --remaining; --c_left; --p_left;
                SN_WAIT_Q1B1();
            } else {
                SN_PK_GROUP0(OFF);
                --remaining; --c_left; --p_left;
                SN_WAIT_B1();
            }
            if constexpr (PRO) asm volatile("s_waitcnt vmcnt(6)" ::: "memory"); else asm volatile("s_waitcnt vmcnt(5)" ::: "memory");
            SN_BARRIER();
            if constexpr (PS) { SN_READOWN(OFF_NEXT, ((SLOT + 1) % 3) * 1024); SN_READB0(OFF_NEXT); }
            else { SN_READS8(((SLOT + 1) % 3) * 1024); SN_READA4(OFF_NEXT); SN_READB0(OFF_NEXT); }
            if constexpr (PS) SN_PMFMA(ql1, ph1); else SN_PMFMA(CP.l, ph1);
            if (!(RING_ABLATE & 1)) {
                const unsigned lds_a = dma_base + (unsigned)(SLOT * STAGE * 4);
                if constexpr (MODE == 1) {
#pragma unroll
                    for (int t = 0; t < 2; ++t) {
                        const float* src = ((a_mask[t] >> l_tap) & 1ull) ? reinterpret_cast<const float*>(reinterpret_cast<const char*>(xb) + a_voff[t]) : zero_page;
                        __builtin_amdgcn_global_load_lds((sn_gbl_ptr_t)src, (sn_lds_ptr_t)(size_t)(lds_a + (unsigned)(t * 4096)), 16, 0, 0);
                    }
                } else {
                    dma16(xb, a_voff[0], lds_a);
                    dma16(xb, a_voff[1], lds_a + 4096u);
                }
                dma16(wb, wimg_voff, lds_a + (unsigned)(BM * BK * 4));
            }
            SN_SB();
            if constexpr (PS) SN_PMFMA(qh1, pl1); else SN_PMFMA(CP.h, pl1);
            if (!(RING_ABLATE & 1)) {
                const unsigned lds_b = dma_base + (unsigned)(SLOT * STAGE * 4 + BM * BK * 4);
                dma16(wb, wimg_voff + 4096u, lds_b + 4096u);
                dma16(wb, wimg_voff + 8192u, lds_b + 8192u);
            }
            if constexpr (PRO) { issue_s(SLOT); scb += BK; }
            xb += BK;
            wb += B_STAGE;
            if constexpr (MODE == 2) {
                if (++l_kw == run_steps) { l_kw = 0; ++l_tap; xb += (p.W + 2 * p.pad) * p.Cin - BK * run_steps; }
            } else {
                l_c0 += BK;
                if (l_c0 == p.Cin) {
                    l_c0 = 0;
                    ++l_tap;
                    xb += ld - p.Cin;
                    if (++l_kw == p.KW) { l_kw = 0; xb += row_jump; }
                }
            }
            SN_SB();
            if constexpr (PS) { SN_PS_GROUP1_TAIL(); } else { SN_PK_GROUP1_TAIL(); }
        }
    };
    using s0 = std::integral_constant<int, 0>;
    using s1 = std::integral_constant<int, 1>;
    using s2 = std::integral_constant<int, 2>;
    while (true) {
        if constexpr (PK) {
            int nf = (pt < t_end) ? min(min(c_left, p_left) - 1, remaining - 2) : 0;
            for (; nf >= 3; nf -= 3) { fast_step(s0{}); fast_step(s1{}); fast_step(s2{}); }
        }
        if (!step(s0{})) break;
        if (!step(s1{})) break;
        if (!step(s2{})) break;
    }
#undef SN_BARRIER
#undef SN_DS_READ
#undef SN_READ0
#undef SN_READ1
#undef SN_WAIT0
#undef SN_WAIT1
#undef SN_MFMA1
#undef SN_READ0P
#undef SN_READ1P
#undef SN_WAIT0P
#undef SN_WAIT1P
#undef SN_PRO
#undef SN_READA
#undef SN_READB0
#undef SN_READB1
#undef SN_READS8
#undef SN_WAIT_A01
#undef SN_WAIT_A23B0
#undef SN_WAIT_B1
#undef SN_READA4
#undef SN_SB
#undef SN_PMFMA
#undef SN_L1
#undef SN_L2
#undef SN_L3
#undef SN_READQ
#undef SN_WAIT_Q0B0
#undef SN_WAIT_Q1B1
#undef SN_READOWN
#undef SN_WRITEQ
#undef SN_PS_GROUP0
#undef SN_PS_GROUP1_TAIL
#undef SN_PK_GROUP0
#undef SN_PK_GROUP1_TAIL
}
```

### deep-online-video-stabilization_amd/ops.py

```python
from __future__ import annotations

import numpy as np
import torch

from . import _lib
from ._tensor import dev_f32, empty, ptr, stream_ptr


def pack_conv_weight(w_hwio, cin_pad: int = 16) -> np.ndarray:
    w = np.asarray(w_hwio, np.float32)
    kh, kw, ci, co = w.shape
    cp = -(-ci // cin_pad) * cin_pad
    out = np.zeros((co, kh, kw, cp), np.float32)
    out[..., :ci] = np.transpose(w, (3, 0, 1, 2))
    return out


def unpack_conv_weight(w_ohwi, cin: int) -> np.ndarray:
    return np.ascontiguousarray(np.transpose(np.asarray(w_ohwi, np.float32)[..., :cin], (1, 2, 3, 0)))


def conv2d(x, w_ohwi, bias=None, in_scale=None, in_shift=None, residual=None, res_stride=1, stride=1, pad=0,
           relu_out=False, out_scale=None, out_shift=None):
    x = dev_f32(x, "x")
    w = dev_f32(w_ohwi, "w")
    N, H, W, Cin = x.shape
    Cout, KH, KW, Cw = w.shape
    assert Cw == Cin, "weight Cin %d != input Cin %d" % (Cw, Cin)
    Ho = (H + 2 * pad - KH) // stride + 1
    Wo = (W + 2 * pad - KW) // stride + 1
    y = empty((N, Ho, Wo, Cout), x)
    L = _lib.lib()
    ws_bytes = L.stabnet_conv2d_workspace_bytes(N, H, W, Cin, Cout, KH, KW, stride, pad)
    ws = torch.empty(max(ws_bytes, 4), dtype=torch.uint8, device=x.device)
    rH, rW = (residual.shape[1], residual.shape[2]) if residual is not None else (0, 0)
    _lib.call("stabnet_conv2d_fwd_ex", ptr(x), ptr(w), ptr(bias), ptr(in_scale), ptr(in_shift), ptr(residual), rH, rW,
              res_stride, ptr(out_scale), ptr(out_shift), ptr(y), N, H, W, Cin, Cout, KH, KW, stride, pad,
              int(relu_out), ptr(ws), ws_bytes, stream_ptr(x.device), device=x.device)
    return y


def conv2d_packed(x, w_ohwi, bias=None, in_scale=None, in_shift=None, residual=None, res_stride=1, stride=1, pad=0,
                  relu_out=False, out_scale=None, out_shift=None, splitk=0):
    x = dev_f32(x, "x")
    w = dev_f32(w_ohwi, "w")
    N, H, W, Cin = x.shape
    Cout, KH, KW, Cw = w.shape
    assert Cw == Cin, "weight Cin %d != input Cin %d" % (Cw, Cin)
    Ho = (H + 2 * pad - KH) // stride + 1
    Wo = (W + 2 * pad - KW) // stride + 1
    y = empty((N, Ho, Wo, Cout), x)
    L = _lib.lib()
    n_img = int(L.stabnet_conv_weight_image_floats(Cout, KH, KW, Cin))
    img = torch.empty(max(n_img, 1), dtype=torch.float32, device=x.device)
    if n_img > 0:
        _lib.call("stabnet_conv_weight_split_image", ptr(w), Cout, KH, KW, Cin, ptr(img), stream_ptr(x.device), device=x.device)
    ws_bytes = max(int(L.stabnet_conv2d_workspace_bytes(N, H, W, Cin, Cout, KH, KW, stride, pad)), max(splitk, 0) * N * Ho * Wo * Cout * 4)
    ws = torch.empty(max(ws_bytes, 4), dtype=torch.uint8, device=x.device)
    rH, rW = (residual.shape[1], residual.shape[2]) if residual is not None else (0, 0)
    _lib.call("stabnet_conv2d_fwd_packed", ptr(x), ptr(w), ptr(img), ptr(bias), ptr(in_scale), ptr(in_shift), ptr(residual), rH, rW,
              res_stride, ptr(out_scale), ptr(out_shift), ptr(y), N, H, W, Cin, Cout, KH, KW, stride, pad, int(relu_out), int(splitk),
              ptr(ws), ws_bytes, stream_ptr(x.device), device=x.device)
    return y


def conv3x3_conv1x1(x, w2_ohwi, mid_scale, mid_shift, w3_ohwi, bias3=None, residual=None, res_stride=1, stride=1, relu_out=False,
                    out_scale=None, out_shift=None, x_ch0=0, res_ch0=0):
    x = dev_f32(x, "x")
    w2 = dev_f32(w2_ohwi, "w2")
    w3 = dev_f32(w3_ohwi, "w3")
    N, H, W, Cx = x.shape
    C = w2.shape[0]
    Cout = w3.shape[0]
    assert tuple(w2.shape) == (C, 3, 3, C) and tuple(w3.shape[1:]) == (1, 1, C) and x_ch0 + C <= Cx
    Ho = (H + 2 - 3) // stride + 1
    Wo = (W + 2 - 3) // stride + 1
    y = empty((N, Ho, Wo, Cout), x)
    rH = rW = res_ld = 0
    rp = 0
    if residual is not None:
        residual = dev_f32(residual, "residual")
        rH, rW, res_ld = residual.shape[1], residual.shape[2], residual.shape[3]
        assert res_ch0 + Cout <= res_ld
        rp = residual.data_ptr() + 4 * res_ch0
    _lib.call("stabnet_conv3x3_conv1x1_fwd", x.data_ptr() + 4 * x_ch0, Cx, ptr(w2), ptr(mid_scale), ptr(mid_shift), ptr(w3),
              ptr(bias3), rp, rH, rW, res_stride, res_ld, ptr(out_scale), ptr(out_shift), ptr(y), N, H, W, C, Cout, stride,
              int(relu_out), stream_ptr(x.device), device=x.device)
    return y


def conv2d_wgrad(x, dy, w_shape, in_scale=None, in_shift=None, stride=1, pad=0, dw=None):
    x = dev_f32(x, "x")
    dy = dev_f32(dy, "dy")
    N, H, W, Cin = x.shape
    Cout, KH, KW, Cw = w_shape
    assert Cw == Cin
    if dw is None:
        dw = torch.zeros(w_shape, dtype=torch.float32, device=x.device)
    nbytes = _lib.lib().stabnet_conv2d_wgrad_workspace_bytes(N, H, W, Cin, Cout, KH, KW, stride, pad)
    ws = torch.empty(nbytes, dtype=torch.uint8, device=x.device)
    _lib.call("stabnet_conv2d_wgrad", ptr(x), ptr(dy), ptr(dw), ptr(in_scale), ptr(in_shift), N, H, W, Cin, Cout, KH, KW,
              stride, pad, ptr(ws), nbytes, stream_ptr(x.device), device=x.device)
    return dw


def conv2d_wgrad_bias(x, dy, w_shape, in_scale=None, in_shift=None, dw=None, db=None):
    x = dev_f32(x, "x")
    dy = dev_f32(dy, "dy")
    N, H, W, Cin = x.shape
    Cout = w_shape[0]
    assert tuple(w_shape[1:]) == (1, 1, Cin)
    buf = torch.zeros(Cout * Cin + Cout, dtype=torch.float32, device=x.device)
    if dw is not None:
        buf[:Cout * Cin] = dw.reshape(-1)
    if db is not None:
        buf[Cout * Cin:] = db
    nbytes = _lib.lib().stabnet_conv2d_wgrad_bias_workspace_bytes(N, H, W, Cin, Cout)
    ws = torch.empty(nbytes, dtype=torch.uint8, device=x.device)
    _lib.call("stabnet_conv2d_wgrad_bias", ptr(x), ptr(dy), buf.data_ptr(), buf.data_ptr() + 4 * Cout * Cin, ptr(in_scale), ptr(in_shift),
              N, H, W, Cin, Cout, ptr(ws), nbytes, stream_ptr(x.device), device=x.device)
    return buf[:Cout * Cin].reshape(w_shape), buf[Cout * Cin:]


def conv2d_wgrad_rowrun(x, dy, w_shape, stride=1, pad=0, dw=None):
    x = dev_f32(x, "x")
    dy = dev_f32(dy, "dy")
    N, H, W, Cin = x.shape
    Cout, KH, KW, CinPad = w_shape
    if dw is None:
        dw = torch.zeros(w_shape, dtype=torch.float32, device=x.device)
    nbytes = _lib.lib().stabnet_conv2d_wgrad_rowrun_workspace_bytes(N, H, W, Cin, Cout, KH, KW, stride, pad)
    ws = torch.empty(nbytes, dtype=torch.uint8, device=x.device)
    _lib.call("stabnet_conv2d_wgrad_rowrun", ptr(x), ptr(dy), ptr(dw), N, H, W, Cin, CinPad, Cout, KH, KW, stride, pad,
              ptr(ws), nbytes, stream_ptr(x.device), device=x.device)
    return dw


def conv2d_dgrad(dy, w_ohwi, x_shape, stride=1, pad=0, residual=None):
    dy = dev_f32(dy, "dy")
    w = dev_f32(w_ohwi, "w")
    N, H, W, Cin = x_shape
    Cout, KH, KW, _ = w.shape
    dx = torch.empty(x_shape, dtype=torch.float32, device=dy.device)
    L = _lib.lib()
    nbytes = L.stabnet_conv2d_dgrad_workspace_bytes(N, H, W, Cin, Cout, KH, KW, stride, pad)
    ws = torch.empty(nbytes, dtype=torch.uint8, device=dy.device)
    _lib.call("stabnet_conv2d_dgrad", ptr(dy), ptr(w), ptr(dx), ptr(residual), N, H, W, Cin, Cout, KH, KW, stride, pad,
              ptr(ws), nbytes, stream_ptr(dy.device), device=dy.device)
    return dx
```

### include/stabnet_hip.h

```cpp
#ifndef STABNET_HIP_H
#define STABNET_HIP_H

#include <stddef.h>
#include <stdint.h>

#ifdef __cplusplus
extern "C" {
#endif

const char* stabnet_last_error(void);
int stabnet_abi_version(void);


int stabnet_get_4_pts(const float* theta, int N, int grid_h, int grid_w, float do_crop_rate,
                      float* pts1, float* pts2, float* Hs, void* stream);

int stabnet_transformer_fwd(const float* pts2, const float* U, int N, int H, int W, int C, int grid_h, int grid_w,
                            float* out, float* black, float* x_map, float* y_map, float* Hs, void* stream);

int stabnet_warp_fwd(const float* theta, const float* U, int N, int H, int W, int C, int grid_h, int grid_w,
                     float do_crop_rate, float* out, float* black, float* x_map, float* y_map, float* Hs,
                     float* pts2, void* stream);

int stabnet_maps_from_hs_fwd(const float* Hs, const float* U, int N, int H, int W, int C, int grid_h, int grid_w,
                             float* out, float* black, float* x_map, float* y_map, void* stream);

int stabnet_interp_fwd(const float* im, const float* x, const float* y, int N, int H, int W, int C, float* out,
                       void* stream);


size_t stabnet_conv2d_workspace_bytes(int N, int H, int W, int Cin, int Cout, int KH, int KW, int stride, int pad);
void stabnet_conv_tuning_override(int tile, int splitk);
void stabnet_conv_tuning_table_set(int M, int Cout, int K, int KH, int ring, int splitk);
void stabnet_conv_tuning_profile(int profile);
int stabnet_conv2d_fwd(const float* x, const float* w_ohwi, const float* bias, const float* in_scale,
                       const float* in_shift, const float* residual, int res_H, int res_W, int res_stride, float* y,
                       int N, int H, int W, int Cin, int Cout, int KH, int KW, int stride, int pad, int relu_out,
                       void* workspace, size_t workspace_bytes, void* stream);
int stabnet_conv2d_fwd_ex(const float* x, const float* w_ohwi, const float* bias, const float* in_scale,
                          const float* in_shift, const float* residual, int res_H, int res_W, int res_stride,
                          const float* out_scale, const float* out_shift, float* y, int N, int H, int W, int Cin,
                          int Cout, int KH, int KW, int stride, int pad, int relu_out, void* workspace,
                          size_t workspace_bytes, void* stream);
size_t stabnet_conv_weight_image_floats(int Cout, int KH, int KW, int Cin);
int stabnet_conv_weight_split_image(const float* w_ohwi, int Cout, int KH, int KW, int Cin, float* w_img, void* stream);
int stabnet_conv2d_fwd_packed(const float* x, const float* w_ohwi, const float* w_img, const float* bias, const float* in_scale,
                              const float* in_shift, const float* residual, int res_H, int res_W, int res_stride,
                              const float* out_scale, const float* out_shift, float* y, int N, int H, int W, int Cin,
                              int Cout, int KH, int KW, int stride, int pad, int relu_out, int splitk, void* workspace,
                              size_t workspace_bytes, void* stream);
int stabnet_conv3x3_conv1x1_fwd(const float* x, int x_ld, const float* w2_ohwi, const float* mid_scale, const float* mid_shift,
                                const float* w3_ohwi, const float* bias3, const float* residual, int res_H, int res_W,
                                int res_stride, int res_ld, const float* out_scale, const float* out_shift, float* y, int N, int H,
                                int W, int C, int Cout, int stride, int relu_out, void* stream);

int stabnet_net_create(void** net, int N, int H, int W, int in_ch, int n_theta, int keep_activations);
void stabnet_net_destroy(void* net);
int stabnet_net_set_bf16_operands(void* net, int on);
int stabnet_net_num_params(const void* net);
int stabnet_net_param_info(const void* net, int idx, char* name, int name_cap, long* offset, int* kind, int* dims4,
                           int* aux);
size_t stabnet_net_param_floats(const void* net);
size_t stabnet_net_trainable_floats(const void* net);
size_t stabnet_net_bn_channels(const void* net);
size_t stabnet_net_workspace_bytes(const void* net);
double stabnet_net_flops(const void* net);
int stabnet_net_num_launches(const void* net);
int stabnet_deploy_frame_launches(const void* net, int grid_h, int grid_w);
int stabnet_net_activation_info(const void* net, const char* name, long* offset, int* dims4);

int stabnet_net_fold_bn(const void* net, const float* params, float* fold, float eps, void* stream);
size_t stabnet_net_fold_floats(const void* net);

int stabnet_backbone_fwd_infer(const void* net, const float* params, const float* fold, const float* x_tensor,
                               float* theta, void* workspace, size_t workspace_bytes, void* stream, void* prof);


int stabnet_ring_init(float* frames_ring, float* masks_ring, const float* first_frame, int S, int depth, int H, int W,
                      void* stream);

int stabnet_deploy_frame(const void* net, const float* params, const float* fold, float* frames_ring,
                         float* masks_ring, int depth, int* head, const int* lags, int n_lags, const float* cur_frame,
                         int refine, int grid_h, int grid_w, float do_crop_rate, float* theta, float* out_img,
                         float* black, float* x_map, float* y_map, float* Hs, float* frame_fb, int* all_black,
                         void* workspace, size_t workspace_bytes, void* stream, void* prof);

int stabnet_prof_create(void** prof, int max_records);
void stabnet_prof_destroy(void* prof);
int stabnet_prof_reset(void* prof);
int stabnet_prof_record_empty(void* prof, void* stream);
int stabnet_prof_num_records(const void* prof);
int stabnet_prof_record(const void* prof, int idx, int* kind, float* ms, double* flops, double* bytes);
int stabnet_prof_record_shape(const void* prof, int idx, int* shape4);
const char* stabnet_prof_kind_name(int kind);

int stabnet_probe_mfma_f32(float* out , int blocks, int iters,
                           unsigned long long* stamps ,
                           void* stream);
double stabnet_probe_mfma_f32_flops(int blocks, int iters);
int stabnet_probe_hbm_copy(const float* src, float* dst, long n_floats, void* stream);
int stabnet_probe_comm_proxy(const float* src, float* dst, long n_floats, int workgroups, int lds_bytes, unsigned long long* stamps,
                             void* stream);
int stabnet_conv_reserve_cus(int reserved);


int stabnet_transformer_bwd(const float* pts2, const float* Hs, const float* U, const float* x_map, const float* y_map,
                            const float* d_out, const float* d_xmap, const float* d_ymap, const float* dmap_scale, int N,
                            int H, int W, int C, int grid_h, int grid_w, float* d_pts2, void* workspace, void* stream);

int stabnet_interp_bwd(const float* x, const float* y, const float* d_out, int N, int H, int W, int C, float* d_im,
                       int accumulate, void* workspace, void* stream);

int stabnet_slice_channel(const float* x, long npix, int C, int c, float* out, void* stream);
int stabnet_interleave2(const float* a, const float* b, long n, float* out, void* stream);

int stabnet_axpb(const float* x, float a, float b, long n, float* y, void* stream);

size_t stabnet_masked_mse_workspace_bytes(int N);
int stabnet_masked_mse_sums(const float* a, const float* b, const float* black, const float* m2, int N, long hw,
                            float* sums, void* workspace, void* stream);
int stabnet_masked_mse_grad(const float* a, const float* b, const float* black, const float* m2, const float* sums,
                            float coef, int N, long hw, float* ga, int accumulate_a, float* gb, void* stream);

int stabnet_feature_loss(const float* matches, const float* mask, const float* x_map, const float* y_map, int N, int H,
                         int W, int max_matches, float gcoef, float* value, float* d_xmap, float* d_ymap, float* dscale,
                         float* warped, void* stream);

int stabnet_mesh_losses(const float* theta, const float* d_pts2_warp, int N, int grid_h, int grid_w, float do_crop_rate,
                        float id_mul, float w_id, float w_dist, float w_cons, float use_black, float w_black,
                        float* losses4, float* d_theta, void* stream);


size_t stabnet_conv2d_wgrad_workspace_bytes(int N, int H, int W, int Cin, int Cout, int KH, int KW, int stride, int pad);
int stabnet_conv2d_wgrad(const float* x, const float* dy, float* dw, const float* in_scale, const float* in_shift,
                         int N, int H, int W, int Cin, int Cout, int KH, int KW, int stride, int pad, void* workspace,
                         size_t workspace_bytes, void* stream);

size_t stabnet_conv2d_wgrad_bias_workspace_bytes(int N, int H, int W, int Cin, int Cout);
int stabnet_conv2d_wgrad_bias(const float* x, const float* dy, float* dw, float* d_bias, const float* in_scale, const float* in_shift,
                              int N, int H, int W, int Cin, int Cout, void* workspace, size_t workspace_bytes, void* stream);

size_t stabnet_conv2d_wgrad_rowrun_workspace_bytes(int N, int H, int W, int Cin, int Cout, int KH, int KW, int stride, int pad);
int stabnet_conv2d_wgrad_rowrun(const float* x, const float* dy, float* dw, int N, int H, int W, int Cin, int CinPad, int Cout,
                                int KH, int KW, int stride, int pad, void* workspace, size_t workspace_bytes, void* stream);

size_t stabnet_conv2d_dgrad_workspace_bytes(int N, int H, int W, int Cin, int Cout, int KH, int KW, int stride, int pad);
int stabnet_conv2d_dgrad(const float* dy, const float* w_ohwi, float* dx, const float* residual, int N, int H, int W,
                         int Cin, int Cout, int KH, int KW, int stride, int pad, void* workspace,
                         size_t workspace_bytes, void* stream);

size_t stabnet_net_train_workspace_bytes(const void* net);

int stabnet_tower_fwd_train(const void* net, float* params, const float* x_tensor, float* theta, void* workspace,
                            size_t workspace_bytes, float bn_eps, float bn_decay, void* stream, void* prof);

int stabnet_towers_fwd_train(const void* net, float* params, const float* x1, const float* x2, float* theta1, float* theta2,
                             void* workspace1, void* workspace2, size_t workspace_bytes, float bn_eps, float bn_decay,
                             void* stream, void* prof);

int stabnet_tower_bwd(const void* net, const float* params, const float* d_theta, float* grads, void* workspace,
                      size_t workspace_bytes, void* stream, void* prof);
int stabnet_tower_bwd_stage(const void* net, const float* params, const float* d_theta, float* grads, void* workspace,
                            size_t workspace_bytes, int stage, void* stream, void* prof);
int stabnet_towers_bwd_stage(const void* net, const float* params, const float* d_theta1, const float* d_theta2, float* grads,
                             void* workspace1, void* workspace2, size_t workspace_bytes, int stage, void* stream, void* prof);
int stabnet_net_num_grad_stages(void);
int stabnet_net_grad_bucket(const void* net, int stage, long* lo, long* hi);
int stabnet_net_bn_grad_range(const void* net, long* lo, long* hi);

int stabnet_net_train_bn_offsets(const void* net, long* scale_off, long* shift_off, long* mean_off, long* invstd_off);

int stabnet_net_train_debug_offset(const void* net, const char* what, long* off, long* count);

int stabnet_weight_decay(const float* params, float* grads, const long* seg_off, const long* seg_len,
                         const float* seg_coef, int nseg, float gscale, float* loss_out, float* workspace, void* stream);

int stabnet_adam_step(float* params, const float* grads, const float* grads2, float* m, float* v, long n, float lr,
                      float beta1, float beta2, float eps, int step, float gscale, void* stream);

int stabnet_warp_rev_bundle2(const unsigned char* img, const float* x_map, const float* y_map, int N, int H, int W, int C,
                             int rate, unsigned char* out, float* workspace, float* px_out, float* py_out, void* stream);

int stabnet_cvt_train2img(const float* x, unsigned char* out, long n, void* stream);

int stabnet_black_accumulate(const float* black, int* all_black, long n, void* stream);
size_t stabnet_crop_search_workspace_bytes(int H, int W, int step);
int stabnet_crop_search(const int* all_black, int H, int W, int step, int* ans5, void* workspace, size_t workspace_bytes,
                        void* stream);

size_t stabnet_augment_workspace_bytes(int N, int H, int W, int before_ch);
int stabnet_augment_pairs(const float* stable, const float* unstable, const float* flow_in, const float* matches1,
                          const int* n1, const float* matches2, const int* n2, const int* para, const float* jitter,
                          const float* Hs, int N, int H, int W, int before_ch, int max_matches, float random_crop_rate,
                          float* x1, float* y1, float* x2, float* y2, float* flow_out, float* fm1, float* mk1, float* fm2,
                          float* mk2, void* workspace, size_t workspace_bytes, void* stream);

#ifdef __cplusplus
}
#endif
#endif
```

Before: 695.3 frames/s.

## Add 128x64 output tile variant to packed bf16x3 ring conv kernel

Adds a WIDE template mode to the packed split-MFMA ring conv kernel. Each wave now owns 32 rows and both 32-column halves, so one A fragment feeds two MFMA accumulators and the B weight image is loaded into a separate double-buffered region shared across the whole K ring. The launcher picks the wide tile by default whenever the count of 128x64 tiles still fills the resident workgroup slots, which halves B traffic per output and raises MFMA reuse of the A fragments. The cost is more LDS (about 84 KiB), more VGPRs (hard-coded v[180:203] registers) and fewer tiles for load balancing. A tile-forcing API and Python hook are added for testing.

```diff
diff --git a/deep-online-video-stabilization_amd/csrc/conv.hip b/deep-online-video-stabilization_amd/csrc/conv.hip
--- a/deep-online-video-stabilization_amd/csrc/conv.hip
+++ b/deep-online-video-stabilization_amd/csrc/conv.hip
@@ -257,6 +257,15 @@
     return share ? 5 : 4;
 }
 
+static thread_local int g_packed_tile_force = -1;
+
+static bool packed_wide(const ConvArgs& a, int resident) {
+    static const int on = env_int("STABNET_CONV_PACKED_WIDE", 1);
+    if (conv_packed_variant() != 4) return false;
+    if (g_packed_tile_force >= 0) return g_packed_tile_force == 1;
+    return on == 2 || (on == 1 && (long)cdiv(a.M, 128) * cdiv(a.Cout, 64) * a.splitk >= resident);
+}
+
 template <int MODE>
 static int launch_ring_packed_mode(const ConvArgs& a, hipStream_t st) {
     const int cus = device_cus();
@@ -265,8 +274,16 @@
         return STABNET_ERR_LAUNCH;
     }
     static const int per_cu = env_int("STABNET_CONV_PACKED_WGS_PER_CU", 2);
+    const long resident = (long)per_cu * usable_cus(cus);
+    if (packed_wide(a, (int)resident)) {
+        const int grid = (int)std::min<long>((long)cdiv(a.M, 128) * cdiv(a.Cout, 64) * a.splitk, resident);
+        if (MODE == 0 && a.in_scale != nullptr) conv_ring_f32_kernel<0, 4, 1, 1, 1><<<grid, 256, 0, st>>>(a);
+        else conv_ring_f32_kernel<MODE, 4, 1, 0, 1><<<grid, 256, 0, st>>>(a);
+        SN_LAUNCH_CHECK("conv_ring_f32_kernel<packed, 128 x 64>");
+        return STABNET_OK;
+    }
     const long ntiles = (long)cdiv(a.M, 64) * cdiv(a.Cout, 64) * a.splitk;
-    const int grid = (int)std::min<long>(ntiles, (long)per_cu * usable_cus(cus));
+    const int grid = (int)std::min<long>(ntiles, resident);
     if constexpr (MODE == 0) {
         if (a.in_scale != nullptr) {
             if (conv_packed_variant() == 5) conv_ring_f32_kernel<0, 5, 1, 1><<<grid, 256, 0, st>>>(a);
@@ -785,6 +802,20 @@
     return conv_launch(a, (hipStream_t)stream, nullptr, 4, w_img);
 }
 
+int stabnet_conv2d_fwd_packed_tile(const float* x, const float* w_ohwi, const float* w_img, const float* bias, const float* in_scale,
+                                   const float* in_shift, const float* residual, int res_H, int res_W, int res_stride,
+                                   const float* out_scale, const float* out_shift, float* y, int N, int H, int W, int Cin,
+                                   int Cout, int KH, int KW, int stride, int pad, int relu_out, int splitk, void* workspace,
+                                   size_t workspace_bytes, int tile, void* stream) {
+    SN_REQUIRE(tile >= -1 && tile <= 1, "conv2d_fwd_packed_tile: tile=%d (-1 the plan's, 0 64 x 64, 1 128 x 64)", tile);
+    g_packed_tile_force = tile;
+    const int rc = stabnet_conv2d_fwd_packed(x, w_ohwi, w_img, bias, in_scale, in_shift, residual, res_H, res_W, res_stride, out_scale,
+                                             out_shift, y, N, H, W, Cin, Cout, KH, KW, stride, pad, relu_out, splitk, workspace,
+                                             workspace_bytes, stream);
+    g_packed_tile_force = -1;
+    return rc;
+}
+
 int stabnet_conv3x3_conv1x1_fwd(const float* x, int x_ld, const float* w2_ohwi, const float* mid_scale, const float* mid_shift,
                                 const float* w3_ohwi, const float* bias3, const float* residual, int res_H, int res_W,
                                 int res_stride, int res_ld, const float* out_scale, const float* out_shift, float* y, int N, int H,
diff --git a/deep-online-video-stabilization_amd/csrc/conv_ring_kernel.h b/deep-online-video-stabilization_amd/csrc/conv_ring_kernel.h
--- a/deep-online-video-stabilization_amd/csrc/conv_ring_kernel.h
+++ b/deep-online-video-stabilization_amd/csrc/conv_ring_kernel.h
@@ -26,25 +26,30 @@
 template <int MODE ,
           int BF16 = 0 ,
           int KG = 1 ,
-          int PRO = 0 >
+          int PRO = 0 ,
+          int WIDE = 0 >
 __global__ __launch_bounds__(256 * KG) void conv_ring_f32_kernel(const ConvArgs p) {
-    constexpr int BM = 64, BN = 64, BK = 32;
+    constexpr int BM = WIDE ? 128 : 64, BN = 64, BK = 32;
+    constexpr int NA = BM / 32;
     constexpr bool PK = (BF16 >= 4);
     constexpr bool PS = (BF16 == 5);
 
     constexpr int B_STAGE = PK ? 3072 : BN * BK;
-    constexpr int STAGE = BM * BK + B_STAGE;
+    constexpr int STAGE = BM * BK + (WIDE ? 0 : B_STAGE);
     constexpr int PLANE_FLOATS = (BF16 == 5) ? 3072 : 0;
-    constexpr int GROUP_FLOATS = 3 * STAGE + PLANE_FLOATS;
+    constexpr int GROUP_FLOATS = 3 * STAGE + (WIDE ? 2 * B_STAGE : 0) + PLANE_FLOATS;
     static_assert(!PRO || (MODE == 0 && BF16 != 1), "the fragment prologue exists for the 1x1 fp32 / split kernels");
     static_assert(!PK || KG <= 2, "the packed split kernel splits K inside the workgroup two ways at most (60 KiB of ring per group)");
+    static_assert(!WIDE || (BF16 == 4 && KG == 1), "the 128 x 64 tile exists for the packed split kernel without K groups (84 KiB of ring)");
+    constexpr int VM_STAGE = NA + (PK ? 3 : 2) + (PRO ? 1 : 0);
+    constexpr int VM_WAIT = WIDE ? NA + (PRO ? 1 : 0) : VM_STAGE;
     constexpr int SC_FLOATS = PRO ? 3 * 4 * 64 : 0;
     __shared__ __attribute__((aligned(16))) float ring[KG * GROUP_FLOATS + KG * SC_FLOATS];
 
     const int tid = threadIdx.x, lane = tid & 63, wave = (KG > 1) ? ((tid >> 6) & 3) : (tid >> 6);
     const int grp = (KG > 1) ? __builtin_amdgcn_readfirstlane(tid >> 8) : 0;
     SN_STAMP(0); SN_STAMP_RT(4);
-    const int wm = wave >> 1, wn = wave & 1;
+    const int wm = WIDE ? wave : wave >> 1, wn = WIDE ? 0 : wave & 1;
     const int tiles_m = (p.M + BM - 1) / BM, tiles_n = (p.Cout + BN - 1) / BN;
     const int tiles_mn = tiles_m * tiles_n;
     const int ntiles = (KG > 1) ? tiles_mn : tiles_mn * p.splitk;
@@ -78,8 +83,8 @@
 
     int pt = t_first;
     int p_left = 0;
-    unsigned a_voff[2], w_voff[2];
-    unsigned long long a_mask[2];
+    unsigned a_voff[NA], w_voff[NA];
+    unsigned long long a_mask[NA];
     int l_tap = 0, l_c0 = 0, l_kw = 0;
     const float *xb = p.x, *wb = p.w;
     const float* scb = p.in_scale;
@@ -94,7 +99,7 @@
         if constexpr (MODE == 2) {
             const int Wp = p.W + 2 * p.pad, Hp = p.H + 2 * p.pad;
 #pragma unroll
-            for (int t = 0; t < 2; ++t) {
+            for (int t = 0; t < NA; ++t) {
                 const int row = 8 * (wave + 4 * t) + rr;
                 const int cl = cp ^ ((row >> 1) & 7);
                 const int mc = min(m0 + row, p.M - 1);
@@ -108,7 +113,7 @@
             }
         } else {
 #pragma unroll
-            for (int t = 0; t < 2; ++t) {
+            for (int t = 0; t < NA; ++t) {
                 const int row = 8 * (wave + 4 * t) + rr;
                 const int cl = cp ^ ((row >> 1) & 7);
                 const int m = m0 + row;
@@ -180,6 +185,14 @@
         }
     };
     const unsigned wimg_voff = (unsigned)(wave * 1024 + lane * 16);
+    const float* wb_pend = p.w;
+    bool b_pend = false;
+    unsigned bw_cur = dma_base + (unsigned)(3 * STAGE * 4);
+    const unsigned bw_sum = 2u * bw_cur + (unsigned)(B_STAGE * 4);
+    auto issue_bp = [&](int t) {
+        if (!b_pend || (RING_ABLATE & 1)) return;
+        dma16(wb_pend, wimg_voff + (unsigned)(t * 4096), bw_cur + (unsigned)(t * 4096));
+    };
     auto issue_b = [&](int slot, int t) {
         if (pt >= t_end || (RING_ABLATE & 1)) return;
         if constexpr (PK) dma16(wb, wimg_voff + (unsigned)(t * 4096), dma_base + (unsigned)(slot * STAGE * 4 + BM * BK * 4 + t * 4096));
@@ -208,8 +221,15 @@
         }
     };
     auto issue_part = [&](int slot, int part) {
-        if (part == 0) issue_a(slot, 0);
-        else if (part == 1) { issue_a(slot, 1); issue_b(slot, 0); }
+        if constexpr (WIDE) {
+            if (part == 0) { issue_bp(0); issue_bp(1); }
+            else if (part == 1) { issue_bp(2); issue_a(slot, 0); issue_a(slot, 2); }
+            else if (part == 2) { issue_a(slot, 1); issue_a(slot, 3); if constexpr (PRO) issue_s(slot); }
+            else { b_pend = pt < t_end; wb_pend = wb; issue_advance(); }
+            return;
+        }
+        if (part == 0) { issue_a(slot, 0); if constexpr (WIDE) issue_a(slot, 2); }
+        else if (part == 1) { issue_a(slot, 1); if constexpr (WIDE) issue_a(slot, 3); issue_b(slot, 0); }
         else if (part == 2) { issue_b(slot, 1); if constexpr (PK) issue_b(slot, 2); if constexpr (PRO) issue_s(slot); }
         else issue_advance();
     };
@@ -243,9 +263,11 @@
         }
     }
 
-    f32x16 acc[1][1];
-#pragma unroll
-    for (int r = 0; r < 16; ++r) acc[0][0][r] = 0.f;
+    f32x16 acc[1][1 + WIDE];
+#pragma unroll
+    for (int j = 0; j <= WIDE; ++j)
+#pragma unroll
+        for (int r = 0; r < 16; ++r) acc[0][j][r] = 0.f;
 
     if (remaining == 0) return;
     producer_setup();
@@ -370,6 +392,56 @@
     SN_PMFMA(CP.h, pm1); SN_L2(AP, x, y0, y1); SN_L2(AP, y, y2, y3); SN_SB();                                            \
     SN_PMFMA(CP.h, ph1); SN_L2(AP, z, y4, y5); SN_L2(AP, w, y6, y7);                                                     \
     SN_L3(AP, x, y0, y1); SN_L3(AP, y, y2, y3); SN_L3(AP, z, y4, y5); SN_L3(AP, w, y6, y7); SN_SB()
+#define SN_PH0W "{v[180:183]}"
+#define SN_PM0W "{v[184:187]}"
+#define SN_PL0W "{v[188:191]}"
+#define SN_PH1W "{v[192:195]}"
+#define SN_PM1W "{v[196:199]}"
+#define SN_PL1W "{v[200:203]}"
+#define SN_READB0W()                                                                                                      \
+    do {                                                                                                                  \
+        SN_DS_READ(ph0, SN_PH0, bfr_cur, 0); SN_DS_READ(pm0, SN_PM0, bfr_cur, 2048); SN_DS_READ(pl0, SN_PL0, bfr_cur, 4096); \
+        SN_DS_READ(ph0w, SN_PH0W, bfr_cur, 6144); SN_DS_READ(pm0w, SN_PM0W, bfr_cur, 8192); SN_DS_READ(pl0w, SN_PL0W, bfr_cur, 10240); \
+    } while (0)
+#define SN_READB1W()                                                                                                      \
+    do {                                                                                                                  \
+        SN_DS_READ(ph1, SN_PH1, bfr_cur, 1024); SN_DS_READ(pm1, SN_PM1, bfr_cur, 3072); SN_DS_READ(pl1, SN_PL1, bfr_cur, 5120); \
+        SN_DS_READ(ph1w, SN_PH1W, bfr_cur, 7168); SN_DS_READ(pm1w, SN_PM1W, bfr_cur, 9216); SN_DS_READ(pl1w, SN_PL1W, bfr_cur, 11264); \
+    } while (0)
+#define SN_TIE_B0W() asm volatile("" : "+" SN_PH0W(ph0w), "+" SN_PM0W(pm0w), "+" SN_PL0W(pl0w))
+#define SN_TIE_B1W() asm volatile("" : "+" SN_PH1W(ph1w), "+" SN_PM1W(pm1w), "+" SN_PL1W(pl1w))
+#define SN_PMFMAW(ap, breg) do { if (!(RING_ABLATE & 8)) acc[0][WIDE] = __builtin_amdgcn_mfma_f32_32x32x16_bf16(__builtin_bit_cast(sn_bf16x8, ap), __builtin_bit_cast(sn_bf16x8, breg), acc[0][WIDE], 0, 0, 0); else acc[0][WIDE][0] += __builtin_bit_cast(float, ap.x) + breg.x; SN_SB(); } while (0)
+#define SN_PK_GROUP0W(OFF_)                                                                                              \
+    SN_READB1W();                                                                                                        \
+    SN_WAIT_A23B0(6); SN_TIE_B0W();                                                                                      \
+    if constexpr (PRO) { SN_PRO(a2, sc2, sh2); SN_PRO(a3, sc3, sh3); }                                                   \
+    float x0 = a2.x, x1 = a2.y, x2 = a2.z, x3 = a2.w, x4 = a3.x, x5 = a3.y, x6 = a3.z, x7 = a3.w;                        \
+    SN_SB();                                                                                                             \
+    SN_PMFMA(AP.l, ph0); SN_L1(CP, x, x0, x1); SN_SB();                                                                  \
+    SN_PMFMAW(AP.l, ph0w); SN_L1(CP, y, x2, x3); SN_SB();                                                                \
+    SN_PMFMA(AP.h, pl0); SN_L1(CP, z, x4, x5); SN_SB();                                                                  \
+    SN_PMFMAW(AP.h, pl0w); SN_L1(CP, w, x6, x7); SN_SB();                                                                \
+    SN_PMFMA(AP.m, pm0); SN_L2(CP, x, x0, x1); SN_SB();                                                                  \
+    SN_PMFMAW(AP.m, pm0w); SN_L2(CP, y, x2, x3); SN_SB();                                                                \
+    SN_PMFMA(AP.m, ph0); SN_L2(CP, z, x4, x5); SN_SB();                                                                  \
+    SN_PMFMAW(AP.m, ph0w); SN_L2(CP, w, x6, x7); SN_SB();                                                                \
+    SN_PMFMA(AP.h, pm0); SN_L3(CP, x, x0, x1); SN_L3(CP, y, x2, x3); SN_SB();                                            \
+    SN_PMFMAW(AP.h, pm0w); SN_L3(CP, z, x4, x5); SN_L3(CP, w, x6, x7); SN_SB();                                          \
+    SN_PMFMA(AP.h, ph0);                                                                                                 \
+    SN_PMFMAW(AP.h, ph0w)
+#define SN_PK_GROUP1_TAILW()                                                                                             \
+    SN_WAIT_A01(8);                                         \
+    if constexpr (PRO) { SN_PRO(a0, sc0, sh0); SN_PRO(a1, sc1, sh1); }                                                   \
+    float y0 = a0.x, y1 = a0.y, y2 = a0.z, y3 = a0.w, y4 = a1.x, y5 = a1.y, y6 = a1.z, y7 = a1.w;                        \
+    SN_SB();                                                                                                             \
+    SN_PMFMA(CP.m, pm1); SN_L1(AP, x, y0, y1); SN_SB();                                                                  \
+    SN_PMFMAW(CP.m, pm1w); SN_L1(AP, y, y2, y3); SN_SB();                                                                \
+    SN_PMFMA(CP.m, ph1); SN_L1(AP, z, y4, y5); SN_SB();                                                                  \
+    SN_PMFMAW(CP.m, ph1w); SN_L1(AP, w, y6, y7); SN_SB();                                                                \
+    SN_PMFMA(CP.h, pm1); SN_L2(AP, x, y0, y1); SN_L2(AP, y, y2, y3); SN_SB();                                            \
+    SN_PMFMAW(CP.h, pm1w); SN_L2(AP, z, y4, y5); SN_L2(AP, w, y6, y7); SN_SB();                                          \
+    SN_PMFMA(CP.h, ph1); SN_L3(AP, x, y0, y1); SN_L3(AP, y, y2, y3); SN_SB();                                            \
+    SN_PMFMAW(CP.h, ph1w); SN_L3(AP, z, y4, y5); SN_L3(AP, w, y6, y7); SN_SB()
 #define SN_RS0 "{v[116:119]}"
 #define SN_RH0 "{v[120:123]}"
 #define SN_RS1 "{v[124:127]}"
@@ -404,12 +476,15 @@
     f32x4 a2, a3;
     f32x4 sc2, sh2, sc3, sh3;
     SnPlanes AP, CP;
+    f32x4 ph0w, pm0w, pl0w, ph1w, pm1w, pl1w;
     f32x4 qh0, qm0, ql0, qh1, qm1, ql1;
     const unsigned pl_base = lds_base + (unsigned)(3 * STAGE * 4);
     const unsigned pl_rd0 = pl_base + (unsigned)((wm * 2 + 0) * 3072 + lane * 16), pl_rd1 = pl_base + (unsigned)((wm * 2 + 1) * 3072 + lane * 16);
     const unsigned pl_wr = pl_base + (unsigned)((wm * 2 + wn) * 3072 + lane * 16);
     unsigned a_own0 = 0u, a_own1 = 0u, s_own0 = 0u, s_own1 = 0u;
     const unsigned bimg_frag = lds_base + (unsigned)(4 * BM * BK + wn * 6144 + lane * 16);
+    unsigned bfr_cur = lds_base + (unsigned)(3 * STAGE * 4 + lane * 16);
+    const unsigned bfr_sum = 2u * bfr_cur + (unsigned)(B_STAGE * 4);
     unsigned s_frag[4] = {0u, 0u, 0u, 0u};
     if constexpr (PRO) {
 #pragma unroll
@@ -425,9 +500,22 @@
         }
     }
     if (RING_ABLATE & 4) { a0 = b0 = a1 = b1 = f32x4{1.f, 2.f, 3.f, 4.f}; }
-    issue(0);
-    issue(1);
-    if (remaining > 1) { if constexpr (PRO && PK) asm volatile("s_waitcnt vmcnt(6)" ::: "memory"); else if constexpr (PRO || PK) asm volatile("s_waitcnt vmcnt(5)" ::: "memory"); else asm volatile("s_waitcnt vmcnt(4)" ::: "memory"); }
+    if constexpr (WIDE) {
+        for (int s = 0; s < 2; ++s) {
+            if (pt < t_end && !(RING_ABLATE & 1)) {
+#pragma unroll
+                for (int t = 0; t < 3; ++t) dma16(wb, wimg_voff + (unsigned)(t * 4096), (s ? bw_sum - bw_cur : bw_cur) + (unsigned)(t * 4096));
+            }
+#pragma unroll
+            for (int t = 0; t < NA; ++t) issue_a(s, t);
+            if constexpr (PRO) issue_s(s);
+            issue_advance();
+        }
+    } else {
+        issue(0);
+        issue(1);
+    }
+    if (remaining > 1) asm volatile("s_waitcnt vmcnt(%0)" ::"n"(VM_STAGE) : "memory");
     else asm volatile("s_waitcnt vmcnt(0)" ::: "memory");
     SN_BARRIER();
     SN_STAMP(1);
@@ -439,6 +527,12 @@
         const SnPlanes NP0 = sn_split3_pair(a0, a1);
         SN_SB();
         SN_WRITEQ(NP0);
+        SN_SB();
+    } else if constexpr (PK && WIDE) {
+        SN_READS8(0); SN_READA4(0); SN_READB0W();
+        SN_WAIT_A01(8);
+        if constexpr (PRO) { SN_PRO(a0, sc0, sh0); SN_PRO(a1, sc1, sh1); }
+        AP = sn_split3_pair(a0, a1);
         SN_SB();
     } else if constexpr (PK) {
         SN_READS8(0); SN_READA4(0); SN_READB0(0);
@@ -473,23 +567,27 @@
             if (feed) { issue_part(SLOT, 2); issue_part(SLOT, 3); SN_SB(); }
             SN_PS_GROUP1_TAIL();
         } else if constexpr (PK) {
-            SN_PK_GROUP0(OFF);
+            if constexpr (WIDE) { SN_PK_GROUP0W(OFF); } else { SN_PK_GROUP0(OFF); }
             --remaining;
             tile_done = (--c_left == 0);
             more = remaining > 0;
             const bool feed = more && !tile_done;
             SN_WAIT_B1();
+            if constexpr (WIDE) SN_TIE_B1W();
             if (more) {
-                if (remaining > 1) { if constexpr (PRO) asm volatile("s_waitcnt vmcnt(6)" ::: "memory"); else asm volatile("s_waitcnt vmcnt(5)" ::: "memory"); }
+                if (remaining > 1) asm volatile("s_waitcnt vmcnt(%0)" ::"n"(VM_WAIT) : "memory");
                 else asm volatile("s_waitcnt vmcnt(0)" ::: "memory");
                 SN_BARRIER();
             }
-            SN_READS8(((SLOT + 1) % 3) * 1024); SN_READA4(OFF_NEXT); SN_READB0(OFF_NEXT);
+            SN_READS8(((SLOT + 1) % 3) * 1024); SN_READA4(OFF_NEXT);
+            if constexpr (WIDE) { bfr_cur = bfr_sum - bfr_cur; SN_READB0W(); } else SN_READB0(OFF_NEXT);
             SN_PMFMA(CP.l, ph1);
+            if constexpr (WIDE) SN_PMFMAW(CP.l, ph1w);
             if (feed) { issue_part(SLOT, 0); issue_part(SLOT, 1); SN_SB(); }
             SN_PMFMA(CP.h, pl1);
+            if constexpr (WIDE) SN_PMFMAW(CP.h, pl1w);
             if (feed) { issue_part(SLOT, 2); issue_part(SLOT, 3); SN_SB(); }
-            SN_PK_GROUP1_TAIL();
+            if constexpr (WIDE) { SN_PK_GROUP1_TAILW(); } else { SN_PK_GROUP1_TAIL(); }
         } else if constexpr (BF16 >= 2) {
             constexpr int NPROD = (BF16 == 3) ? 9 : 6;
             constexpr int SOFF = SLOT * 1024, SOFF_NEXT = ((SLOT + 1) % 3) * 1024;
@@ -634,7 +732,7 @@
         }
         if (tile_done) {
             if constexpr (PS) { asm volatile("s_waitcnt lgkmcnt(0)" : "+" SN_PH0(ph0), "+" SN_PM0(pm0), "+" SN_PL0(pl0)); if (!more) SN_BARRIER(); }
-            else if constexpr (PK) { SN_WAIT_A23B0(0); if (!more) SN_BARRIER(); }
+            else if constexpr (PK) { SN_WAIT_A23B0(0); if constexpr (WIDE) SN_TIE_B0W(); if (!more) SN_BARRIER(); }
             else if (more) { if constexpr (PRO) SN_WAIT0P(); else SN_WAIT0(); }
             else SN_BARRIER();
             SN_STAMP(2);
@@ -666,17 +764,19 @@
                                               lds_base + (unsigned)(OFF + wave * SN_EPI_WAVE_BYTES));
                 }
             } else if constexpr (PRO)
-            conv_epilogue<1, 1, false, true>(acc, p, c_m0 + wm * 32, c_n0 + wn * 32, lane, c_z,
-                                             lds_base + (unsigned)(OFF + wave * SN_EPI_WAVE_BYTES), c_yoff, c_roff);
+            conv_epilogue<1, 1 + WIDE, false, true>(acc, p, c_m0 + wm * 32, c_n0 + wn * 32, lane, c_z,
+                                                    lds_base + (unsigned)(OFF + wave * SN_EPI_WAVE_BYTES), c_yoff, c_roff);
             else
-            conv_epilogue<1, 1>(acc, p, c_m0 + wm * 32, c_n0 + wn * 32, lane, c_z,
-                                lds_base + (unsigned)(OFF + wave * SN_EPI_WAVE_BYTES));
+            conv_epilogue<1, 1 + WIDE>(acc, p, c_m0 + wm * 32, c_n0 + wn * 32, lane, c_z,
+                                       lds_base + (unsigned)(OFF + wave * SN_EPI_WAVE_BYTES));
 #if RING_STAMP
             asm volatile("s_waitcnt vmcnt(0)" ::: "memory");
             SN_STAMP(3); SN_STAMP_RT(5);
 #endif
 #pragma unroll
-            for (int r = 0; r < 16; ++r) acc[0][0][r] = 0.f;
+            for (int j = 0; j <= WIDE; ++j)
+#pragma unroll
+                for (int r = 0; r < 16; ++r) acc[0][j][r] = 0.f;
             ct += t_stride;
             if (ct < t_end) consumer_setup();
             if (more) {
@@ -684,6 +784,7 @@
                 issue(SLOT);
             }
         }
+        if constexpr (WIDE) bw_cur = bw_sum - bw_cur;
         return more;
     };
     auto fast_step = [&](auto slot_c) {
@@ -696,27 +797,41 @@
                 --remaining; --c_left; --p_left;
                 SN_WAIT_Q1B1();
             } else {
-                SN_PK_GROUP0(OFF);
+                if constexpr (WIDE) { SN_PK_GROUP0W(OFF); } else { SN_PK_GROUP0(OFF); }
                 --remaining; --c_left; --p_left;
                 SN_WAIT_B1();
-            }
-            if constexpr (PRO) asm volatile("s_waitcnt vmcnt(6)" ::: "memory"); else asm volatile("s_waitcnt vmcnt(5)" ::: "memory");
+                if constexpr (WIDE) SN_TIE_B1W();
+            }
+            asm volatile("s_waitcnt vmcnt(%0)" ::"n"(VM_WAIT) : "memory");
             SN_BARRIER();
             if constexpr (PS) { SN_READOWN(OFF_NEXT, ((SLOT + 1) % 3) * 1024); SN_READB0(OFF_NEXT); }
+            else if constexpr (WIDE) { bfr_cur = bfr_sum - bfr_cur; SN_READS8(((SLOT + 1) % 3) * 1024); SN_READA4(OFF_NEXT); SN_READB0W(); }
             else { SN_READS8(((SLOT + 1) % 3) * 1024); SN_READA4(OFF_NEXT); SN_READB0(OFF_NEXT); }
             if constexpr (PS) SN_PMFMA(ql1, ph1); else SN_PMFMA(CP.l, ph1);
+            const unsigned lds_a = dma_base + (unsigned)(SLOT * STAGE * 4);
+            auto dma_a = [&](int t) {
+                if constexpr (MODE == 1) {
+                    const float* src = ((a_mask[t] >> l_tap) & 1ull) ? reinterpret_cast<const float*>(reinterpret_cast<const char*>(xb) + a_voff[t]) : zero_page;
+                    __builtin_amdgcn_global_load_lds((sn_gbl_ptr_t)src, (sn_lds_ptr_t)(size_t)(lds_a + (unsigned)(t * 4096)), 16, 0, 0);
+                } else {
+                    dma16(xb, a_voff[t], lds_a + (unsigned)(t * 4096));
+                }
+            };
+            if constexpr (WIDE) {
+                if (!(RING_ABLATE & 1)) { dma16(wb_pend, wimg_voff, bw_cur); dma16(wb_pend, wimg_voff + 4096u, bw_cur + 4096u); }
+                SN_SB();
+                SN_PMFMAW(CP.l, ph1w);
+                if (!(RING_ABLATE & 1)) { dma16(wb_pend, wimg_voff + 8192u, bw_cur + 8192u); dma_a(0); dma_a(2); }
+                SN_SB();
+                SN_PMFMA(CP.h, pl1);
+                if (!(RING_ABLATE & 1)) { dma_a(1); dma_a(3); }
+                SN_SB();
+                SN_PMFMAW(CP.h, pl1w);
+                wb_pend = wb;
+            } else {
             if (!(RING_ABLATE & 1)) {
-                const unsigned lds_a = dma_base + (unsigned)(SLOT * STAGE * 4);
-                if constexpr (MODE == 1) {
-#pragma unroll
-                    for (int t = 0; t < 2; ++t) {
-                        const float* src = ((a_mask[t] >> l_tap) & 1ull) ? reinterpret_cast<const float*>(reinterpret_cast<const char*>(xb) + a_voff[t]) : zero_page;
-                        __builtin_amdgcn_global_load_lds((sn_gbl_ptr_t)src, (sn_lds_ptr_t)(size_t)(lds_a + (unsigned)(t * 4096)), 16, 0, 0);
-                    }
-                } else {
-                    dma16(xb, a_voff[0], lds_a);
-                    dma16(xb, a_voff[1], lds_a + 4096u);
-                }
+                dma_a(0);
+                dma_a(1);
                 dma16(wb, wimg_voff, lds_a + (unsigned)(BM * BK * 4));
             }
             SN_SB();
@@ -725,6 +840,7 @@
                 const unsigned lds_b = dma_base + (unsigned)(SLOT * STAGE * 4 + BM * BK * 4);
                 dma16(wb, wimg_voff + 4096u, lds_b + 4096u);
                 dma16(wb, wimg_voff + 8192u, lds_b + 8192u);
+            }
             }
             if constexpr (PRO) { issue_s(SLOT); scb += BK; }
             xb += BK;
@@ -741,7 +857,7 @@
                 }
             }
             SN_SB();
-            if constexpr (PS) { SN_PS_GROUP1_TAIL(); } else { SN_PK_GROUP1_TAIL(); }
+            if constexpr (PS) { SN_PS_GROUP1_TAIL(); } else if constexpr (WIDE) { SN_PK_GROUP1_TAILW(); bw_cur = bw_sum - bw_cur; } else { SN_PK_GROUP1_TAIL(); }
         }
     };
     using s0 = std::integral_constant<int, 0>;
@@ -790,4 +906,11 @@
 #undef SN_PS_GROUP1_TAIL
 #undef SN_PK_GROUP0
 #undef SN_PK_GROUP1_TAIL
+#undef SN_READB0W
+#undef SN_READB1W
+#undef SN_TIE_B0W
+#undef SN_TIE_B1W
+#undef SN_PMFMAW
+#undef SN_PK_GROUP0W
+#undef SN_PK_GROUP1_TAILW
 }
diff --git a/deep-online-video-stabilization_amd/ops.py b/deep-online-video-stabilization_amd/ops.py
--- a/deep-online-video-stabilization_amd/ops.py
+++ b/deep-online-video-stabilization_amd/ops.py
@@ -41,7 +41,7 @@
 
 
 def conv2d_packed(x, w_ohwi, bias=None, in_scale=None, in_shift=None, residual=None, res_stride=1, stride=1, pad=0,
-                  relu_out=False, out_scale=None, out_shift=None, splitk=0):
+                  relu_out=False, out_scale=None, out_shift=None, splitk=0, tile=None):
     x = dev_f32(x, "x")
     w = dev_f32(w_ohwi, "w")
     N, H, W, Cin = x.shape
@@ -58,9 +58,12 @@
     ws_bytes = max(int(L.stabnet_conv2d_workspace_bytes(N, H, W, Cin, Cout, KH, KW, stride, pad)), max(splitk, 0) * N * Ho * Wo * Cout * 4)
     ws = torch.empty(max(ws_bytes, 4), dtype=torch.uint8, device=x.device)
     rH, rW = (residual.shape[1], residual.shape[2]) if residual is not None else (0, 0)
-    _lib.call("stabnet_conv2d_fwd_packed", ptr(x), ptr(w), ptr(img), ptr(bias), ptr(in_scale), ptr(in_shift), ptr(residual), rH, rW,
-              res_stride, ptr(out_scale), ptr(out_shift), ptr(y), N, H, W, Cin, Cout, KH, KW, stride, pad, int(relu_out), int(splitk),
-              ptr(ws), ws_bytes, stream_ptr(x.device), device=x.device)
+    args = (ptr(x), ptr(w), ptr(img), ptr(bias), ptr(in_scale), ptr(in_shift), ptr(residual), rH, rW, res_stride, ptr(out_scale),
+            ptr(out_shift), ptr(y), N, H, W, Cin, Cout, KH, KW, stride, pad, int(relu_out), int(splitk), ptr(ws), ws_bytes)
+    if tile is None:
+        _lib.call("stabnet_conv2d_fwd_packed", *args, stream_ptr(x.device), device=x.device)
+    else:
+        _lib.call("stabnet_conv2d_fwd_packed_tile", *args, int(tile), stream_ptr(x.device), device=x.device)
     return y
 
 
diff --git a/include/stabnet_hip.h b/include/stabnet_hip.h
--- a/include/stabnet_hip.h
+++ b/include/stabnet_hip.h
@@ -49,6 +49,11 @@
                               const float* out_scale, const float* out_shift, float* y, int N, int H, int W, int Cin,
                               int Cout, int KH, int KW, int stride, int pad, int relu_out, int splitk, void* workspace,
                               size_t workspace_bytes, void* stream);
+int stabnet_conv2d_fwd_packed_tile(const float* x, const float* w_ohwi, const float* w_img, const float* bias, const float* in_scale,
+                                   const float* in_shift, const float* residual, int res_H, int res_W, int res_stride,
+                                   const float* out_scale, const float* out_shift, float* y, int N, int H, int W, int Cin,
+                                   int Cout, int KH, int KW, int stride, int pad, int relu_out, int splitk, void* workspace,
+                                   size_t workspace_bytes, int tile, void* stream);
 int stabnet_conv3x3_conv1x1_fwd(const float* x, int x_ld, const float* w2_ohwi, const float* mid_scale, const float* mid_shift,
                                 const float* w3_ohwi, const float* bias3, const float* residual, int res_H, int res_W,
                                 int res_stride, int res_ld, const float* out_scale, const float* out_shift, float* y, int N, int H,
```

Measured after the change: 702.6 frames/s (median of 6 runs). 1.0% higher.
